# AlexS28/OptiState

Hardware: NVIDIA B200
Metric: kf_trajectory_steps_per_sec (higher is better)
Workload: dtype f64

## Files before the change

### optistate_b200/batch.py

```python
from __future__ import annotations

from dataclasses import dataclass, field
from typing import Dict, Iterable, Optional

import numpy as np
import torch

from . import _native as nv
from .settings import INITIAL_PARAMS

_OUT_ALIASES = {"p_trace": "p_trace_steps", "k_gain": "k_gain_steps", "p_checkpoints": "P_ckpt", "nis": "nis_steps"}
_OUT_SHAPES = {
    "x_steps": lambda T, N, K: (T, 12, N), "x_model_steps": lambda T, N, K: (T, 12, N),
    "p_world_steps": lambda T, N, K: (T, 12, N), "z_steps": lambda T, N, K: (T, 10, N),
    "p_trace_steps": lambda T, N, K: (T, N), "k_gain_steps": lambda T, N, K: (T, N), "nis_steps": lambda T, N, K: (T, N),
    "P_ckpt": lambda T, N, K: (K, 144, N), "x_final": lambda T, N, K: (12, N), "P_final": lambda T, N, K: (144, N),
    "K_final": lambda T, N, K: (120, N), "summary": lambda T, N, K: (nv.SUMMARY_ROWS, N),
}
_ALGOS = {"auto": nv.ALGO_AUTO, "joint": nv.ALGO_JOINT, "sequential": nv.ALGO_SEQUENTIAL}
_ALGO_NAMES = {nv.ALGO_JOINT: "joint", nv.ALGO_SEQUENTIAL: "sequential"}

_GROUP = torch.tensor([0, 0, 0, 1, 2, 3, 0, 0, 0, 1, 2, 3])
_CROSS_GROUP = _GROUP[:, None] != _GROUP[None, :]

SUMMARY_FIELDS = {
    "x_final": slice(0, 12), "p_diag": slice(12, 24), "rmse_truth": slice(24, 36), "rms_dev_nominal": slice(36, 48),
    "mean_nis": 48, "p_trace": 49, "k_gain": 50, "max_nis_sqrt": 51,
}


@dataclass
class KfBatchResult:
    algo: str
    n_traj: int
    n_steps: int
    tensors: Dict[str, torch.Tensor] = field(default_factory=dict)
    status: Optional[torch.Tensor] = None

    def __getattr__(self, name):
        t = self.__dict__.get("tensors", {})
        if name in t:
            return t[name]
        raise AttributeError(name)

    def P_matrix(self, which: str = "P_final") -> torch.Tensor:
        t = self.tensors[which]
        return t.movedim(-1, -2).reshape(*t.shape[:-2], t.shape[-1], 12, 12)

    def summary_field(self, name: str) -> torch.Tensor:
        return self.tensors["summary"][SUMMARY_FIELDS[name]]


def _as_device(a, dtype, device, non_blocking=True):
    if a is None:
        return None
    if isinstance(a, torch.Tensor):
        t = a
    else:
        t = torch.from_numpy(np.ascontiguousarray(a))
    if t.device != device or t.dtype != dtype:
        t = t.to(device=device, dtype=dtype, non_blocking=non_blocking)
    return t.contiguous()


def _stream_tensor(a, C, name, dtype, device):
    t = _as_device(a, dtype, device)
    if t is None:
        return None, None, None
    if t.dim() == 2:
        t = t.unsqueeze(-1)
    if t.dim() != 3 or t.shape[1] != C:
        raise ValueError(f"{name} must have shape [T, {C}, S], got {tuple(t.shape)}")
    return t.contiguous(), t.shape[0], t.shape[2]


def _checked_stream_index(stream_index, N: int, S: int, device) -> torch.Tensor:
    t = _as_device(stream_index, torch.int32, device).reshape(N)
    if N > 0:
        lo, hi = (int(v) for v in torch.aminmax(t))
        if lo < 0 or hi >= S:
            raise ValueError(f"stream_index entries must lie in [0, {S}), got [{lo}, {hi}]")
    return t


def _is_diagonal(m: torch.Tensor) -> bool:
    return bool(torch.count_nonzero(m - torch.diag(torch.diagonal(m))) == 0)


def _noise(a, n, N, name, dtype, device, kind=None):
    t = _as_device(a, dtype, device)
    shp = tuple(t.shape)
    if kind is None:
        if shp == (n,):
            kind = nv.MAT_DIAG
        elif shp == (n, n):
            kind = nv.MAT_DENSE
        elif shp == (n, N):
            kind = nv.MAT_DIAG_PER
        elif shp in ((n * n, N), (n, n, N)):
            kind = nv.MAT_DENSE_PER
        else:
            raise ValueError(f"{name}: unsupported shape {shp} for n={n}, N={N}")
    if kind == nv.MAT_DENSE and _is_diagonal(t.reshape(n, n)):
        t, kind = torch.diagonal(t.reshape(n, n)).contiguous(), nv.MAT_DIAG
    return t.contiguous(), kind


def kf_batch(
    imu, p, dp, contact, f, x0=None, P0=None, Q=None, R=None, *,
    n_traj: Optional[int] = None, dtype: torch.dtype = torch.float64, stream_index=None, stream_offset: int = 0,
    outputs: Iterable[str] = ("x_steps",), ckpt_every: int = 0, truth=None, nominal=None, body_ref=None, z=None,
    algo: str = "auto", cov_model: str = "predict", q_kind=None, r_kind=None, p0_kind=None,
    dt: float = INITIAL_PARAMS.DT_mpc, mass: float = INITIAL_PARAMS.ROBOT_MASS, inertia=None,
    gravity: float = INITIAL_PARAMS.GRAVITY, device=None, out: Optional[Dict[str, torch.Tensor]] = None,
    summary_peers=None, p0_is_symmetric: Optional[bool] = None, structure: str = "auto", packed: bool = True,
) -> KfBatchResult:
    nv.require_cuda()
    ext = nv.ext()
    device = torch.device("cuda", torch.cuda.current_device()) if device is None else torch.device(device)
    if dtype not in (torch.float64, torch.float32):
        raise ValueError("dtype must be torch.float64 or torch.float32")

    tensors: Dict[str, torch.Tensor] = {}
    T = S = None
    for name, arr, C in (("imu", imu, 6), ("p", p, 12), ("dp", dp, 12), ("contact", contact, 4), ("f", f, 12),
                         ("z_in", z, 10), ("body_ref", body_ref, 12), ("truth", truth, 12), ("nominal", nominal, 12)):
        t, tT, tS = _stream_tensor(arr, C, name, dtype, device)
        if t is None:
            continue
        if T is None:
            T, S = tT, tS
        elif (tT, tS) != (T, S):
            raise ValueError(f"{name} has [T,S]=({tT},{tS}), expected ({T},{S})")
        tensors[name] = t
    if T is None:
        raise ValueError("no input streams given")
    N = int(S if n_traj is None else n_traj)
    phases = nv.PHASE_ALL if z is None else (nv.PHASE_PREDICT | nv.PHASE_UPDATE)

    x0_t = _as_device(INITIAL_PARAMS.STARTING_STATE.reshape(12) if x0 is None else x0, dtype, device)
    x0_t = x0_t.reshape(12) if x0_t.numel() == 12 else x0_t.reshape(12, N)
    tensors["x0"] = x0_t.contiguous()
    tensors["Q"], qk = _noise(INITIAL_PARAMS.Q if Q is None else Q, 12, N, "Q", dtype, device, q_kind)
    tensors["R"], rk = _noise(INITIAL_PARAMS.R if R is None else R, 10, N, "R", dtype, device, r_kind)
    pk = nv.MAT_NONE
    p0_symmetric = True
    if structure not in ("auto", "full"):
        raise ValueError("structure must be 'auto' or 'full'")
    flags = nv.FLAG_FULL_COVARIANCE if structure == "full" else 0
    if not packed:
        flags |= nv.FLAG_SCALAR_FP32
    if P0 is not None:
        tensors["P0"], pk = _noise(P0, 12, N, "P0", dtype, device, p0_kind)
        if pk in (nv.MAT_DENSE, nv.MAT_DENSE_PER):
            m = tensors["P0"].reshape(12, 12, -1)
            p0_symmetric = bool(torch.equal(m, m.transpose(0, 1))) if p0_is_symmetric is None else bool(p0_is_symmetric)
            if structure == "auto" and p0_is_symmetric is None and p0_symmetric and cov_model != "mpc":
                if not bool(torch.count_nonzero(m[_CROSS_GROUP.to(device)])):
                    flags |= nv.FLAG_P0_DECOUPLED
    if stream_index is not None:
        tensors["stream_index"] = _checked_stream_index(stream_index, N, S, device)

    want = []
    for o in outputs:
        o = _OUT_ALIASES.get(o, o)
        want.extend(["x_final", "P_final"] if o == "final" else [o])
    n_ckpt = T // ckpt_every if ckpt_every else 0
    for o in want:
        if o not in _OUT_SHAPES:
            raise ValueError(f"unknown output '{o}'")
        shape = _OUT_SHAPES[o](T, N, n_ckpt)
        if o == "summary" and summary_peers is not None:
            if summary_peers.dtype != dtype or summary_peers.n_local != N or summary_peers.device != device:
                raise ValueError("summary_peers was set up for another dtype, device or shard size")
            tensors[o] = summary_peers.tensor
        elif out is not None and o in out:
            if tuple(out[o].shape) != shape or out[o].dtype != dtype:
                raise ValueError(f"out['{o}'] must be {shape} {dtype}")
            tensors[o] = out[o]
        else:
            tensors[o] = torch.empty(shape, dtype=dtype, device=device)
    status = out["status"] if out is not None and "status" in out else torch.zeros(N, dtype=torch.int32, device=device)
    tensors["status"] = status

    cfg = dict(dtype=nv.F64 if dtype == torch.float64 else nv.F32, algo=_ALGOS[algo],
               cov_model=nv.COV_MPC if cov_model == "mpc" else nv.COV_PREDICT, phases=phases, n_traj=N, n_steps=T,
               n_streams=S, stream_offset=int(stream_offset), x0_per_traj=int(x0_t.dim() == 2), p0_kind=pk, q_kind=qk,
               r_kind=rk, ckpt_every=int(ckpt_every), want_K=int("K_final" in want), flags=flags)
    if summary_peers is not None and "summary" in want:
        cfg.update(summary_peers.cfg())
    if cfg["algo"] == nv.ALGO_AUTO:
        probe = dict(cfg, algo=nv.ALGO_SEQUENTIAL)
        cfg["algo"] = nv.ALGO_SEQUENTIAL if (p0_symmetric and ext.kf_resolve_algo(probe) == nv.ALGO_SEQUENTIAL) else nv.ALGO_JOINT
    elif cfg["algo"] == nv.ALGO_SEQUENTIAL and not p0_symmetric:
        raise ValueError("algo='sequential' needs a symmetric P0")
    inertia = np.diag(INITIAL_PARAMS.INERTIA_ROT) if inertia is None else np.asarray(inertia, float).reshape(3)
    consts = dict(dt=float(dt), mass=float(mass), inertia0=float(inertia[0]), inertia1=float(inertia[1]),
                  inertia2=float(inertia[2]), gravity=float(gravity))
    with torch.cuda.device(device):
        ws_bytes = ext.kf_batch(dict(cfg, query_workspace=1), consts, tensors)
        if ws_bytes < 0:
            nv.check(int(ws_bytes), "optistate_kf_workspace_bytes")
        if ws_bytes > 0:
            ws = out.get("workspace") if out is not None else None
            if ws is None or ws.numel() < ws_bytes:
                ws = torch.empty(int(ws_bytes), dtype=torch.uint8, device=device)
            tensors["workspace"] = ws
        nv.check(int(ext.kf_batch(cfg, consts, tensors)), "optistate_kf_batch")
    res = {k: tensors[k] for k in want}
    if summary_peers is not None and "summary" in res:
        res["summary"] = summary_peers.local
    return KfBatchResult(algo=_ALGO_NAMES[cfg["algo"]], n_traj=N, n_steps=T, tensors=res, status=status)


def kf_measure(imu, p, dp, contact, *, dtype: torch.dtype = torch.float64, device=None, want_odom: bool = False):
    nv.require_cuda()
    ext = nv.ext()
    device = torch.device("cuda", torch.cuda.current_device()) if device is None else torch.device(device)
    tensors = {}
    T = S = None
    for name, arr, C in (("imu", imu, 6), ("p", p, 12), ("dp", dp, 12), ("contact", contact, 4)):
        t, tT, tS = _stream_tensor(arr, C, name, dtype, device)
        if T is None:
            T, S = tT, tS
        elif (tT, tS) != (T, S):
            raise ValueError(f"{name} has [T,S]=({tT},{tS}), expected ({T},{S})")
        tensors[name] = t
    tensors["z"] = torch.empty((T, 10, S), dtype=dtype, device=device)
    if want_odom:
        tensors["odom"] = torch.empty((T, 4, S), dtype=dtype, device=device)
    tensors["status"] = torch.zeros(S, dtype=torch.int32, device=device)
    with torch.cuda.device(device):
        nv.check(ext.kf_measure(nv.F64 if dtype == torch.float64 else nv.F32, T, S, tensors), "optistate_kf_measure")
    if want_odom:
        return tensors["z"], tensors["odom"], tensors["status"]
    return tensors["z"], tensors["status"]


def fma_peak(dtype: torch.dtype = torch.float64, fma_per_thread: int = 1 << 16):
    nv.require_cuda()
    return nv.ext().fma_peak(nv.F64 if dtype == torch.float64 else nv.F32, int(fma_per_thread))
```

### optistate_b200/csrc/kf_abi.cu

```cuda
#include <atomic>
#include <cstdlib>
#include <cstring>

#include "kf_features.cuh"
#include "kf_identify.cuh"
#include "kf_launch.cuh"
#include "kf_mpc_params.cuh"

namespace {

std::atomic<long long> g_launches{0};

bool is_diag_kind(int k) { return k == OPTI_KF_MAT_DIAG || k == OPTI_KF_MAT_DIAG_PER; }
bool valid_kind(int k, bool allow_none) { return (k >= (allow_none ? 0 : 1)) && k <= OPTI_KF_MAT_DENSE_PER; }

int validate(const OptiKfDesc *d) {
    if (!d) return OPTI_KF_E_NULL;
    if (d->struct_size != sizeof(OptiKfDesc) || d->abi_version != OPTISTATE_KF_ABI_VERSION) return OPTI_KF_E_VERSION;
    if (d->dtype != OPTI_KF_F64 && d->dtype != OPTI_KF_F32) return OPTI_KF_E_DTYPE;
    if (d->n_traj < 0 || d->n_steps < 0 || d->n_streams <= 0 || d->ckpt_every < 0) return OPTI_KF_E_SHAPE;
    if (d->phases <= 0 || d->phases > OPTI_KF_PHASE_ALL) return OPTI_KF_E_SHAPE;
    if (d->algo < OPTI_KF_ALGO_AUTO || d->algo > OPTI_KF_ALGO_SEQUENTIAL) return OPTI_KF_E_SHAPE;
    if (d->cov_model != OPTI_KF_COV_PREDICT && d->cov_model != OPTI_KF_COV_MPC) return OPTI_KF_E_SHAPE;
    if (!valid_kind(d->q_kind, false) || !valid_kind(d->r_kind, false) || !valid_kind(d->p0_kind, true)) return OPTI_KF_E_SHAPE;
    if (!(d->dt > 0) || !(d->mass > 0) || !(d->inertia[0] > 0) || !(d->inertia[1] > 0) || !(d->inertia[2] > 0)) return OPTI_KF_E_SHAPE;
    const bool work = d->n_traj > 0, steps = work && d->n_steps > 0;
    if (work && (!d->x0 || !d->Q || !d->R)) return OPTI_KF_E_NULL;
    if (work && d->p0_kind != OPTI_KF_MAT_NONE && !d->P0) return OPTI_KF_E_NULL;
    if (steps && (d->phases & OPTI_KF_PHASE_MEASURE) && (!d->imu || !d->p || !d->dp || !d->contact)) return OPTI_KF_E_NULL;
    if (steps && (d->phases & OPTI_KF_PHASE_PREDICT) && (!d->p || !d->f)) return OPTI_KF_E_NULL;
    if (steps && (d->phases & OPTI_KF_PHASE_UPDATE) && !(d->phases & OPTI_KF_PHASE_MEASURE) && !d->z_in) return OPTI_KF_E_NULL;
    if (steps && d->cov_model == OPTI_KF_COV_MPC && (d->phases & OPTI_KF_PHASE_PREDICT) && !d->body_ref) return OPTI_KF_E_NULL;
    if (d->P_ckpt && d->ckpt_every == 0) return OPTI_KF_E_SHAPE;
    if (d->stream_index == nullptr && d->stream_offset < 0) return OPTI_KF_E_SHAPE;
    if (d->summary_ld < 0 || (d->summary_ld > 0 && d->summary_ld < d->n_traj)) return OPTI_KF_E_SHAPE;
    if (d->n_summary_peers < 0 || d->n_summary_peers > OPTI_KF_MAX_PEERS) return OPTI_KF_E_SHAPE;
    if (d->flags & ~(OPTI_KF_FLAG_P0_DECOUPLED | OPTI_KF_FLAG_FULL_COVARIANCE | OPTI_KF_FLAG_SCALAR_FP32 | OPTI_KF_FLAG_STATUS_ACCUMULATE)) return OPTI_KF_E_SHAPE;
    for (int k = 0; k < d->n_summary_peers; ++k)
        if (d->summary && !d->summary_peers[k]) return OPTI_KF_E_NULL;
    return OPTI_KF_OK;
}

bool sequential_ok(const OptiKfDesc *d) {
    return is_diag_kind(d->q_kind) && is_diag_kind(d->r_kind) && d->K_final == nullptr &&
           (d->phases == OPTI_KF_PHASE_ALL || (d->phases == (OPTI_KF_PHASE_PREDICT | OPTI_KF_PHASE_UPDATE) && d->z_in));
}

int resolve(const OptiKfDesc *d) {
    if (d->algo == OPTI_KF_ALGO_JOINT) return OPTI_KF_ALGO_JOINT;
    if (d->algo == OPTI_KF_ALGO_SEQUENTIAL) return sequential_ok(d) ? (int)OPTI_KF_ALGO_SEQUENTIAL : (int)OPTI_KF_E_UNSUPPORTED;
    const bool p0_sym = d->p0_kind == OPTI_KF_MAT_NONE || is_diag_kind(d->p0_kind);
    return (sequential_ok(d) && p0_sym) ? OPTI_KF_ALGO_SEQUENTIAL : OPTI_KF_ALGO_JOINT;
}

template <typename Real>
okf::Params<Real> make_params(const OptiKfDesc *d) {
    okf::Params<Real> p;
    std::memset(&p, 0, sizeof p);
    p.N = d->n_traj; p.T = d->n_steps; p.S = d->n_streams; p.stream_offset = d->stream_offset;
    p.phases = d->phases; p.cov_model = d->cov_model;
    const bool p0_groups = d->p0_kind == OPTI_KF_MAT_NONE || is_diag_kind(d->p0_kind) || (d->flags & OPTI_KF_FLAG_P0_DECOUPLED);
    p.block = (d->cov_model == OPTI_KF_COV_PREDICT && p0_groups && !(d->flags & OPTI_KF_FLAG_FULL_COVARIANCE)) ? 1 : 0;
    p.dt = (Real)d->dt;
    p.dt_over_m = (Real)((1.0 / d->mass) * d->dt);
    p.dt_g = (Real)(d->dt * d->gravity);
    for (int k = 0; k < 3; ++k) p.inv_inertia[k] = (Real)(1.0 / d->inertia[k]);
    p.imu = (const Real *)d->imu; p.p = (const Real *)d->p; p.dp = (const Real *)d->dp;
    p.contact = (const Real *)d->contact; p.f = (const Real *)d->f;
    p.z_in = (d->phases & OPTI_KF_PHASE_MEASURE) ? nullptr : (const Real *)d->z_in;
    p.body_ref = (const Real *)d->body_ref; p.truth = (const Real *)d->truth; p.nominal = (const Real *)d->nominal;
    p.stream_index = d->stream_index;
    p.x0 = (const Real *)d->x0; p.x0_ld = d->x0_per_traj ? d->n_traj : 1; p.x0_inc = d->x0_per_traj ? 1 : 0;
    p.P0 = (const Real *)d->P0; p.p0_kind = d->p0_kind;
    p.Q = (const Real *)d->Q; p.q_kind = d->q_kind;
    p.R = (const Real *)d->R; p.r_kind = d->r_kind;
    p.x_steps = (Real *)d->x_steps; p.x_model_steps = (Real *)d->x_model_steps; p.p_world_steps = (Real *)d->p_world_steps;
    p.z_steps = (Real *)d->z_steps; p.p_trace_steps = (Real *)d->p_trace_steps; p.k_gain_steps = (Real *)d->k_gain_steps;
    p.nis_steps = (Real *)d->nis_steps; p.ckpt_every = d->ckpt_every; p.P_ckpt = (Real *)d->P_ckpt;
    p.x_final = (Real *)d->x_final; p.P_final = (Real *)d->P_final; p.K_final = (Real *)d->K_final;
    p.summary = (Real *)d->summary; p.status = d->status;
    p.summary_ld = d->summary_ld > 0 ? d->summary_ld : d->n_traj;
    p.n_summary_peers = d->summary ? d->n_summary_peers : 0;
    for (int k = 0; k < p.n_summary_peers; ++k) p.summary_peers[k] = (Real *)d->summary_peers[k];
    return p;
}

template <typename Real>
void launch_measure(long long T, long long S, const Real *imu, const Real *p, const Real *dp, const Real *contact, Real *z,
                    Real *odom, uint32_t *status, cudaStream_t stream);

inline bool aligned16(const void *p) { return (reinterpret_cast<uintptr_t>(p) & 15u) == 0; }

size_t seq_workspace_bytes(const OptiKfDesc *d) {
    if (d->phases != OPTI_KF_PHASE_ALL) return 0;
    const size_t esz = d->dtype == OPTI_KF_F64 ? 8 : 4;
    const size_t z_bytes = ((size_t)d->n_steps * okf::NZ * (size_t)d->n_streams * esz + 255) & ~(size_t)255;
    return z_bytes + (((size_t)d->n_streams * sizeof(uint32_t) + 255) & ~(size_t)255);
}

bool tma_layout_ok(const OptiKfDesc *d) {
    if (d->stream_index != nullptr || d->n_steps == 0) return false;
    if (d->n_streams % 32 != 0 || d->stream_offset % 32 != 0) return false;
    if (d->n_steps * 12 >= (1LL << 31)) return false;
    if (!aligned16(d->p) || !aligned16(d->f)) return false;
    if (d->summary && ((d->truth && !aligned16(d->truth)) || (d->nominal && !aligned16(d->nominal)))) return false;
    if (d->cov_model == OPTI_KF_COV_MPC && !aligned16(d->body_ref)) return false;
    return true;
}

inline bool aligned8(const void *p) { return (reinterpret_cast<uintptr_t>(p) & 7u) == 0; }

bool packed_pair_ok(const OptiKfDesc *d) {
    if (d->dtype != OPTI_KF_F32) return false;
    if (d->flags & OPTI_KF_FLAG_SCALAR_FP32) return false;
    if (d->n_traj % 2 != 0 || d->n_streams % 64 != 0 || d->stream_offset % 64 != 0) return false;
    const void *ptrs[] = {d->x0, d->P0, d->Q, d->R, d->x_steps, d->x_model_steps, d->p_world_steps, d->z_steps, d->p_trace_steps,
                          d->k_gain_steps, d->nis_steps, d->P_ckpt, d->x_final, d->P_final, d->summary};
    for (const void *q : ptrs)
        if (q && !aligned8(q)) return false;
    if (d->summary && d->summary_ld % 2 != 0) return false;
    for (int k = 0; k < d->n_summary_peers; ++k)
        if (d->summary && !aligned8(d->summary_peers[k])) return false;
    return true;
}

template <typename Real>
int launch_streamed_t(const OptiKfDesc *d, const okf::Params<typename okf::Lanes<Real>::scalar> &p, cudaStream_t stream) {
    if constexpr (okf::Lanes<Real>::n == 1) {
        if (p.block && p.N <= p.S && p.cov_model == OPTI_KF_COV_PREDICT)
            return d->summary ? okf::launch_seq_tma_lone<Real, true>(p, stream) : okf::launch_seq_tma_lone<Real, false>(p, stream);
    }
    if (p.block) return d->summary ? okf::launch_seq_tma<Real, true, true>(p, stream) : okf::launch_seq_tma<Real, false, true>(p, stream);
    return d->summary ? okf::launch_seq_tma<Real, true, false>(p, stream) : okf::launch_seq_tma<Real, false, false>(p, stream);
}
template <typename Scalar>
int launch_streamed(const OptiKfDesc *d, const okf::Params<Scalar> &p, cudaStream_t stream);
template <>
int launch_streamed<double>(const OptiKfDesc *d, const okf::Params<double> &p, cudaStream_t stream) {
    return launch_streamed_t<double>(d, p, stream);
}
template <>
int launch_streamed<float>(const OptiKfDesc *d, const okf::Params<float> &p, cudaStream_t stream) {
    return packed_pair_ok(d) ? launch_streamed_t<okf::F2>(d, p, stream) : launch_streamed_t<float>(d, p, stream);
}

template <typename Real>
int launch(const OptiKfDesc *d, int algo, cudaStream_t stream) {
    if (d->n_traj == 0) return OPTI_KF_OK;
    okf::Params<Real> p = make_params<Real>(d);
    cudaGetLastError();
    if ((d->flags & OPTI_KF_FLAG_STATUS_ACCUMULATE) && d->status) {
        if (d->stream_index != nullptr || d->n_streams != d->n_traj || d->stream_offset != 0 || d->phases == OPTI_KF_PHASE_ALL) return OPTI_KF_E_UNSUPPORTED;
        p.stream_status = d->status;
    }
    if (algo == OPTI_KF_ALGO_SEQUENTIAL) {
        bool streamed = tma_layout_ok(d);
        if (streamed && d->phases == OPTI_KF_PHASE_ALL) {
            const size_t need = seq_workspace_bytes(d);
            if (d->workspace && d->workspace_bytes >= need && aligned16(d->workspace)) {
                const size_t esz = sizeof(Real);
                const size_t z_bytes = ((size_t)d->n_steps * okf::NZ * (size_t)d->n_streams * esz + 255) & ~(size_t)255;
                Real *z = (Real *)d->workspace;
                uint32_t *sst = (uint32_t *)((unsigned char *)d->workspace + z_bytes);
                if (cudaMemsetAsync(sst, 0, (size_t)d->n_streams * sizeof(uint32_t), stream) != cudaSuccess) return OPTI_KF_E_CUDA;
                launch_measure<Real>(d->n_steps, d->n_streams, p.imu, p.p, p.dp, p.contact, z, nullptr, sst, stream);
                p.z_in = z;
                p.stream_status = sst;
            } else {
                streamed = false;
            }
        } else if (streamed && !aligned16(p.z_in)) {
            streamed = false;
        }
        if (streamed) {
            const int rc = launch_streamed<Real>(d, p, stream);
            if (rc < 0) return rc;
            if (rc == OPTI_KF_OK) {
                g_launches.fetch_add(1, std::memory_order_relaxed);
                return cudaGetLastError() == cudaSuccess ? OPTI_KF_OK : OPTI_KF_E_CUDA;
            }
        }
        const int rc = okf::launch_seq_direct<Real>(p, stream);
        if (rc < 0) return rc;
    } else {
        const int rc = okf::launch_joint<Real>(p, stream);
        if (rc < 0) return rc;
    }
    g_launches.fetch_add(1, std::memory_order_relaxed);
    return cudaGetLastError() == cudaSuccess ? OPTI_KF_OK : OPTI_KF_E_CUDA;
}

template <typename Real>
__global__ void __launch_bounds__(256) kf_measure_kernel(long long T, long long S, const Real *__restrict__ imu,
                                                         const Real *__restrict__ p, const Real *__restrict__ dp,
                                                         const Real *__restrict__ contact, Real *__restrict__ z,
                                                         Real *__restrict__ odom, uint32_t *__restrict__ status) {
    const long long idx = (long long)blockIdx.x * blockDim.x + threadIdx.x;
    if (idx >= T * S) return;
    const long long t = idx / S, s = idx % S;
    Real im[6], pp[12], dd[12], cc[4], zz[okf::NZ];
#pragma unroll
    for (int c = 0; c < 6; ++c) im[c] = imu[(t * 6 + c) * S + s];
#pragma unroll
    for (int c = 0; c < 12; ++c) { pp[c] = p[(t * 12 + c) * S + s]; dd[c] = dp[(t * 12 + c) * S + s]; }
#pragma unroll
    for (int c = 0; c < 4; ++c) cc[c] = contact[(t * 4 + c) * S + s];
    const bool all_swing = okf::form_measurement(im, pp, dd, cc, zz);
    if (z) {
#pragma unroll
        for (int c = 0; c < okf::NZ; ++c) z[(t * okf::NZ + c) * S + s] = zz[c];
    }
    if (odom) {
        odom[(t * 4 + 0) * S + s] = zz[3];
        odom[(t * 4 + 1) * S + s] = zz[7];
        odom[(t * 4 + 2) * S + s] = zz[8];
        odom[(t * 4 + 3) * S + s] = zz[9];
    }
    if (status && all_swing) atomicOr(status + s, (uint32_t)OPTI_KF_ST_ALL_SWING);
}

template <typename Real>
void launch_measure(long long T, long long S, const Real *imu, const Real *p, const Real *dp, const Real *contact, Real *z,
                    Real *odom, uint32_t *status, cudaStream_t stream) {
    const long long total = T * S;
    if (total == 0) return;
    kf_measure_kernel<Real><<<(unsigned)((total + 255) / 256), 256, 0, stream>>>(T, S, imu, p, dp, contact, z, odom, status);
    g_launches.fetch_add(1, std::memory_order_relaxed);
}

template <typename Real>
__global__ void __launch_bounds__(256) fma_peak_kernel(long long iters, Real seed, Real *sink) {
    Real a[16];
    const Real m = Real(0.999) + seed * Real(1e-9), c = Real(1e-3) * (Real)(threadIdx.x & 7);
#pragma unroll
    for (int k = 0; k < 16; ++k) a[k] = seed + (Real)k;
    for (long long it = 0; it < iters; ++it) {
#pragma unroll
        for (int k = 0; k < 16; ++k) a[k] = a[k] * m + c;
    }
    Real s = Real(0);
#pragma unroll
    for (int k = 0; k < 16; ++k) s += a[k];
    if (s == Real(-12345.678)) sink[blockIdx.x * blockDim.x + threadIdx.x] = s;
}

template <typename Real>
int fma_peak(long long fma_per_thread, double *flops_out, double *seconds_out, cudaStream_t stream) {
    int dev = 0, sms = 0;
    if (cudaGetDevice(&dev) != cudaSuccess) return OPTI_KF_E_NO_DEVICE;
    cudaDeviceGetAttribute(&sms, cudaDevAttrMultiProcessorCount, dev);
    const int blocks = sms * 8, threads = 256;
    const long long iters = (fma_per_thread + 15) / 16;
    cudaEvent_t e0, e1;
    if (cudaEventCreate(&e0) != cudaSuccess || cudaEventCreate(&e1) != cudaSuccess) return OPTI_KF_E_CUDA;
    fma_peak_kernel<Real><<<blocks, threads, 0, stream>>>(iters / 8 + 1, Real(1), nullptr);
    cudaEventRecord(e0, stream);
    fma_peak_kernel<Real><<<blocks, threads, 0, stream>>>(iters, Real(1), nullptr);
    cudaEventRecord(e1, stream);
    g_launches.fetch_add(2, std::memory_order_relaxed);
    if (cudaEventSynchronize(e1) != cudaSuccess) { cudaEventDestroy(e0); cudaEventDestroy(e1); return OPTI_KF_E_CUDA; }
    float ms = 0.f;
    cudaEventElapsedTime(&ms, e0, e1);
    cudaEventDestroy(e0); cudaEventDestroy(e1);
    const double fma = (double)iters * 16.0 * (double)blocks * (double)threads;
    if (flops_out) *flops_out = 2.0 * fma / ((double)ms * 1e-3);
    if (seconds_out) *seconds_out = (double)ms * 1e-3;
    return OPTI_KF_OK;
}

template <typename Real>
int identify_noise(const OptiKfIdentifyDesc *d, cudaStream_t stream) {
    okf::Params<Real> p;
    std::memset(&p, 0, sizeof p);
    p.N = d->n_traj; p.T = d->n_steps; p.S = d->n_streams; p.stream_offset = d->stream_offset; p.stream_index = d->stream_index;
    p.dt = (Real)d->dt;
    p.dt_over_m = (Real)((1.0 / d->mass) * d->dt);
    p.dt_g = (Real)(d->dt * d->gravity);
    for (int k = 0; k < 3; ++k) p.inv_inertia[k] = (Real)(1.0 / d->inertia[k]);
    p.imu = (const Real *)d->imu; p.p = (const Real *)d->p; p.dp = (const Real *)d->dp;
    p.contact = (const Real *)d->contact; p.f = (const Real *)d->f; p.status = d->status;
    const long long pairs = (d->n_steps - 1) * d->n_traj;
    okf::kf_identify_residuals_kernel<Real><<<(unsigned)((pairs + 127) / 128), 128, 0, stream>>>(p, (const Real *)d->gt, d->alias_last_measurement,
                                                                                                  (Real *)d->scratch);
    const long long comps = (long long)okf::IDENT_ROWS * d->n_traj;
    okf::kf_identify_variance_kernel<Real><<<(unsigned)((comps + 127) / 128), 128, 0, stream>>>(d->n_traj, d->n_steps - 1, (const Real *)d->scratch,
                                                                                                 (Real *)d->q_diag, (Real *)d->r_diag);
    g_launches.fetch_add(2, std::memory_order_relaxed);
    return cudaGetLastError() == cudaSuccess ? OPTI_KF_OK : OPTI_KF_E_CUDA;
}

}

extern "C" {

int optistate_kf_abi_version(void) { return OPTISTATE_KF_ABI_VERSION; }
size_t optistate_kf_desc_size(void) { return sizeof(OptiKfDesc); }
int64_t optistate_kf_launch_count(void) { return (int64_t)g_launches.load(std::memory_order_relaxed); }

int optistate_kf_resolve_algo(const OptiKfDesc *desc) {
    const int rc = validate(desc);
    return rc != OPTI_KF_OK ? rc : resolve(desc);
}

int optistate_kf_workspace_bytes(const OptiKfDesc *desc, size_t *bytes_out) {
    const int rc = validate(desc);
    if (rc != OPTI_KF_OK) return rc;
    if (!bytes_out) return OPTI_KF_E_NULL;
    const int algo = resolve(desc);
    if (algo < 0) return algo;
    *bytes_out = (algo == OPTI_KF_ALGO_SEQUENTIAL && tma_layout_ok(desc)) ? seq_workspace_bytes(desc) : 0;
    return OPTI_KF_OK;
}

int optistate_kf_batch(const OptiKfDesc *desc, void *cuda_stream) {
    const int rc = validate(desc);
    if (rc != OPTI_KF_OK) return rc;
    const int algo = resolve(desc);
    if (algo < 0) return algo;
    cudaStream_t stream = (cudaStream_t)cuda_stream;
    return desc->dtype == OPTI_KF_F64 ? launch<double>(desc, algo, stream) : launch<float>(desc, algo, stream);
}

int optistate_kf_batch_f64(const OptiKfDesc *desc, void *cuda_stream) {
    if (desc && desc->dtype != OPTI_KF_F64) return OPTI_KF_E_DTYPE;
    return optistate_kf_batch(desc, cuda_stream);
}

int optistate_kf_batch_f32(const OptiKfDesc *desc, void *cuda_stream) {
    if (desc && desc->dtype != OPTI_KF_F32) return OPTI_KF_E_DTYPE;
    return optistate_kf_batch(desc, cuda_stream);
}

int optistate_kf_measure(const OptiKfMeasureDesc *d, void *cuda_stream) {
    if (!d) return OPTI_KF_E_NULL;
    if (d->struct_size != sizeof(OptiKfMeasureDesc) || d->abi_version != OPTISTATE_KF_ABI_VERSION) return OPTI_KF_E_VERSION;
    if (d->dtype != OPTI_KF_F64 && d->dtype != OPTI_KF_F32) return OPTI_KF_E_DTYPE;
    if (d->n_steps < 0 || d->n_streams <= 0) return OPTI_KF_E_SHAPE;
    if (!d->imu || !d->p || !d->dp || !d->contact || (!d->z && !d->odom)) return OPTI_KF_E_NULL;
    const long long total = d->n_steps * d->n_streams;
    if (total == 0) return OPTI_KF_OK;
    cudaStream_t stream = (cudaStream_t)cuda_stream;
    cudaGetLastError();
    if (d->dtype == OPTI_KF_F64)
        launch_measure<double>(d->n_steps, d->n_streams, (const double *)d->imu, (const double *)d->p, (const double *)d->dp,
                               (const double *)d->contact, (double *)d->z, (double *)d->odom, d->status, stream);
    else
        launch_measure<float>(d->n_steps, d->n_streams, (const float *)d->imu, (const float *)d->p, (const float *)d->dp,
                              (const float *)d->contact, (float *)d->z, (float *)d->odom, d->status, stream);
    return cudaGetLastError() == cudaSuccess ? OPTI_KF_OK : OPTI_KF_E_CUDA;
}

int optistate_fma_peak(int dtype, int64_t fma_per_thread, double *flops_per_s_out, double *seconds_out, void *cuda_stream) {
    if (fma_per_thread <= 0) return OPTI_KF_E_SHAPE;
    cudaStream_t stream = (cudaStream_t)cuda_stream;
    if (dtype == OPTI_KF_F64) return fma_peak<double>(fma_per_thread, flops_per_s_out, seconds_out, stream);
    if (dtype == OPTI_KF_F32) return fma_peak<float>(fma_per_thread, flops_per_s_out, seconds_out, stream);
    return OPTI_KF_E_DTYPE;
}

int optistate_kf_features(const OptiKfFeatureDesc *d, void *cuda_stream) {
    if (!d) return OPTI_KF_E_NULL;
    if (d->struct_size != sizeof(OptiKfFeatureDesc) || d->abi_version != OPTISTATE_KF_ABI_VERSION) return OPTI_KF_E_VERSION;
    if (d->dtype != OPTI_KF_F64 && d->dtype != OPTI_KF_F32) return OPTI_KF_E_DTYPE;
    if (d->n_traj < 0 || d->n_steps < 0 || d->n_streams <= 0) return OPTI_KF_E_SHAPE;
    if ((d->n_steps + okf::FEAT_STEPS - 1) / okf::FEAT_STEPS > 65535) return OPTI_KF_E_SHAPE;
    if (d->stream_index == nullptr && d->stream_offset < 0) return OPTI_KF_E_SHAPE;
    if (!d->x_steps || !d->p_world_steps || !d->imu || !d->f || !d->dp || !d->rows) return OPTI_KF_E_NULL;
    if (d->n_traj == 0 || d->n_steps == 0) return OPTI_KF_OK;
    cudaStream_t stream = (cudaStream_t)cuda_stream;
    const dim3 grid((unsigned)((d->n_traj + okf::FEAT_TRAJ - 1) / okf::FEAT_TRAJ), (unsigned)((d->n_steps + okf::FEAT_STEPS - 1) / okf::FEAT_STEPS));
    cudaGetLastError();
    if (d->dtype == OPTI_KF_F64)
        okf::kf_features_kernel<double><<<grid, 256, 0, stream>>>(d->n_traj, d->n_steps, d->n_streams, d->stream_offset, d->stream_index,
                                                                  (const double *)d->x_steps, (const double *)d->p_world_steps,
                                                                  (const double *)d->imu, (const double *)d->imu_acc, (const double *)d->f,
                                                                  (const double *)d->dp, (double *)d->rows);
    else
        okf::kf_features_kernel<float><<<grid, 256, 0, stream>>>(d->n_traj, d->n_steps, d->n_streams, d->stream_offset, d->stream_index,
                                                                 (const float *)d->x_steps, (const float *)d->p_world_steps,
                                                                 (const float *)d->imu, (const float *)d->imu_acc, (const float *)d->f,
                                                                 (const float *)d->dp, (float *)d->rows);
    g_launches.fetch_add(1, std::memory_order_relaxed);
    return cudaGetLastError() == cudaSuccess ? OPTI_KF_OK : OPTI_KF_E_CUDA;
}

static const int kMinmaxBlocks = 592;
static int sm_count() {
    int dev = 0, n = 0;
    if (cudaGetDevice(&dev) != cudaSuccess || cudaDeviceGetAttribute(&n, cudaDevAttrMultiProcessorCount, dev) != cudaSuccess || n <= 0) n = 148;
    return n;
}

size_t optistate_kf_minmax_scratch_bytes(int dtype, int32_t n_cols) {
    return (size_t)kMinmaxBlocks * 2 * (size_t)(n_cols > 0 ? n_cols : 0) * (dtype == OPTI_KF_F64 ? 8 : 4);
}

int optistate_kf_minmax(int dtype, const void *rows, int64_t n_rows, int32_t n_cols, void *min_out, void *max_out, void *scratch,
                        size_t scratch_bytes, void *cuda_stream) {
    if (dtype != OPTI_KF_F64 && dtype != OPTI_KF_F32) return OPTI_KF_E_DTYPE;
    if (!rows || !min_out || !max_out || !scratch) return OPTI_KF_E_NULL;
    if (n_rows <= 0 || n_cols <= 0 || n_cols > 256 || scratch_bytes < optistate_kf_minmax_scratch_bytes(dtype, n_cols)) return OPTI_KF_E_SHAPE;
    cudaStream_t stream = (cudaStream_t)cuda_stream;
    cudaGetLastError();
    const int nblk = 4 * sm_count() < kMinmaxBlocks ? 4 * sm_count() : kMinmaxBlocks;
    if (dtype == OPTI_KF_F64) {
        okf::kf_minmax_partial_kernel<double><<<nblk, 256, 2 * 256 * sizeof(double), stream>>>((const double *)rows, n_rows, n_cols, (double *)scratch);
        okf::kf_minmax_final_kernel<double><<<1, 256, 0, stream>>>((const double *)scratch, nblk, n_cols, (double *)min_out, (double *)max_out);
    } else {
        okf::kf_minmax_partial_kernel<float><<<nblk, 256, 2 * 256 * sizeof(float), stream>>>((const float *)rows, n_rows, n_cols, (float *)scratch);
        okf::kf_minmax_final_kernel<float><<<1, 256, 0, stream>>>((const float *)scratch, nblk, n_cols, (float *)min_out, (float *)max_out);
    }
    g_launches.fetch_add(2, std::memory_order_relaxed);
    return cudaGetLastError() == cudaSuccess ? OPTI_KF_OK : OPTI_KF_E_CUDA;
}

size_t optistate_kf_windows_scratch_bytes(int64_t n_groups, int64_t rows_per_group, int32_t n_cols, int32_t n_latent) {
    if (n_groups <= 0 || rows_per_group <= 0 || n_cols <= 0 || n_latent < 0) return 0;
    return (size_t)n_groups * (size_t)rows_per_group * (size_t)(n_cols + n_latent) * sizeof(float);
}

int optistate_kf_windows(int dtype, const void *rows, const float *latent, const void *mn, const void *mx, int64_t n_groups,
                         int64_t rows_per_group, int32_t n_cols, int32_t n_latent, int32_t seq_len, float *out, void *scratch,
                         size_t scratch_bytes, void *cuda_stream) {
    if (dtype != OPTI_KF_F64 && dtype != OPTI_KF_F32) return OPTI_KF_E_DTYPE;
    if (!rows || !mn || !mx || !out || !scratch || (n_latent > 0 && !latent)) return OPTI_KF_E_NULL;
    if (n_groups <= 0 || seq_len <= 0 || rows_per_group < seq_len || n_cols <= 0 || n_latent < 0) return OPTI_KF_E_SHAPE;
    if (scratch_bytes < optistate_kf_windows_scratch_bytes(n_groups, rows_per_group, n_cols, n_latent)) return OPTI_KF_E_SHAPE;
    cudaStream_t stream = (cudaStream_t)cuda_stream;
    const long long n_rows = n_groups * rows_per_group;
    const int width = n_cols + n_latent;
    float *full = (float *)scratch;
    cudaGetLastError();
    const unsigned nb = (unsigned)sm_count() * 16;
    if (dtype == OPTI_KF_F64)
        okf::kf_normalise_rows_kernel<double><<<nb, 256, 0, stream>>>((const double *)rows, latent, (const double *)mn, (const double *)mx,
                                                                      n_rows, n_cols, n_latent, full);
    else
        okf::kf_normalise_rows_kernel<float><<<nb, 256, 0, stream>>>((const float *)rows, latent, (const float *)mn, (const float *)mx, n_rows,
                                                                     n_cols, n_latent, full);
    const bool vec4 = (width % 4 == 0) && ((reinterpret_cast<uintptr_t>(full) | reinterpret_cast<uintptr_t>(out)) & 15u) == 0;
    if (vec4)
        okf::kf_windows_copy_kernel<float4><<<nb, dim3(64, 4), 0, stream>>>((const float4 *)full, rows_per_group, n_groups, width / 4, seq_len, (float4 *)out);
    else
        okf::kf_windows_copy_kernel<float><<<nb, dim3(64, 4), 0, stream>>>(full, rows_per_group, n_groups, width, seq_len, out);
    g_launches.fetch_add(2, std::memory_order_relaxed);
    return cudaGetLastError() == cudaSuccess ? OPTI_KF_OK : OPTI_KF_E_CUDA;
}

size_t optistate_kf_identify_scratch_bytes(int dtype, int64_t n_traj, int64_t n_steps) {
    if (n_traj <= 0 || n_steps < 2) return 0;
    return (size_t)(n_steps - 1) * okf::IDENT_ROWS * (size_t)n_traj * (dtype == OPTI_KF_F64 ? 8 : 4);
}

int optistate_kf_identify_noise(const OptiKfIdentifyDesc *d, void *cuda_stream) {
    if (!d) return OPTI_KF_E_NULL;
    if (d->struct_size != sizeof(OptiKfIdentifyDesc) || d->abi_version != OPTISTATE_KF_ABI_VERSION) return OPTI_KF_E_VERSION;
    if (d->dtype != OPTI_KF_F64 && d->dtype != OPTI_KF_F32) return OPTI_KF_E_DTYPE;
    if (d->n_traj <= 0 || d->n_steps < 2 || d->n_streams <= 0) return OPTI_KF_E_SHAPE;
    if (d->stream_index == nullptr && d->stream_offset < 0) return OPTI_KF_E_SHAPE;
    if (!(d->dt > 0) || !(d->mass > 0) || !(d->inertia[0] > 0) || !(d->inertia[1] > 0) || !(d->inertia[2] > 0)) return OPTI_KF_E_SHAPE;
    if (!d->gt || !d->imu || !d->p || !d->dp || !d->contact || !d->f || !d->q_diag || !d->r_diag || !d->scratch) return OPTI_KF_E_NULL;
    if (d->scratch_bytes < optistate_kf_identify_scratch_bytes(d->dtype, d->n_traj, d->n_steps)) return OPTI_KF_E_SHAPE;
    cudaGetLastError();
    cudaStream_t stream = (cudaStream_t)cuda_stream;
    return d->dtype == OPTI_KF_F64 ? identify_noise<double>(d, stream) : identify_noise<float>(d, stream);
}

int optistate_kf_mpc_forces(const OptiKfMpcDesc *d, void *cuda_stream) {
    if (!d) return OPTI_KF_E_NULL;
    if (d->struct_size != sizeof(OptiKfMpcDesc) || d->abi_version != OPTISTATE_KF_ABI_VERSION) return OPTI_KF_E_VERSION;
    if (d->dtype != OPTI_KF_F64) return OPTI_KF_E_DTYPE;
    if (d->n_problems < 0 || d->max_free_legs < 0 || d->max_free_legs > 4) return OPTI_KF_E_SHAPE;
    if (!(d->dt > 0) || !(d->mass > 0) || !(d->inertia[0] > 0) || !(d->inertia[1] > 0) || !(d->inertia[2] > 0) || !(d->mu > 0) ||
        !(d->fz_max > 0) || !(d->w_force > 0))
        return OPTI_KF_E_SHAPE;
    for (int k = 0; k < 12; ++k)
        if (!(d->w_state[k] >= 0)) return OPTI_KF_E_SHAPE;
    if (d->n_problems == 0) return OPTI_KF_OK;
    if (!d->x || !d->body_ref || !d->p || !d->contact || !d->forces || !d->status) return OPTI_KF_E_NULL;
    if ((d->warm_set == nullptr) != (d->warm_mult == nullptr)) return OPTI_KF_E_NULL;
    okf::MpcParams p;
    std::memset(&p, 0, sizeof p);
    p.N = d->n_problems;
    p.max_legs = d->max_free_legs == 0 ? 4 : d->max_free_legs;
    p.x = (const double *)d->x; p.body_ref = (const double *)d->body_ref; p.p = (const double *)d->p;
    p.contact = (const double *)d->contact; p.forces = (double *)d->forces; p.status = d->status;
    p.warm_set = d->warm_set; p.warm_mult = (double *)d->warm_mult;
    if (d->solver != 0 && d->solver != 1) return OPTI_KF_E_SHAPE;
    p.solver = d->solver;
    p.max_changes = d->max_changes > 0 ? d->max_changes : 0;
    p.dt = d->dt; p.inv_mass = 1.0 / d->mass; p.gravity = d->gravity; p.mu = d->mu; p.fz_max = d->fz_max; p.w_force = d->w_force;
    for (int k = 0; k < 3; ++k) p.inv_inertia[k] = 1.0 / d->inertia[k];
    for (int k = 0; k < 12; ++k) p.w_state[k] = d->w_state[k];
    cudaGetLastError();
    const int rc = okf::launch_mpc(p, (cudaStream_t)cuda_stream);
    if (rc < 0) return rc;
    g_launches.fetch_add(1, std::memory_order_relaxed);
    return cudaGetLastError() == cudaSuccess ? OPTI_KF_OK : OPTI_KF_E_CUDA;
}

int optistate_kf_peer_alloc(size_t bytes, void **dev_ptr_out) {
    if (!dev_ptr_out || bytes == 0) return OPTI_KF_E_NULL;
    *dev_ptr_out = nullptr;
    return cudaMalloc(dev_ptr_out, bytes) == cudaSuccess ? (int)OPTI_KF_OK : (cudaGetLastError(), (int)OPTI_KF_E_CUDA);
}

int optistate_kf_peer_free(void *dev_ptr) {
    if (!dev_ptr) return OPTI_KF_OK;
    return cudaFree(dev_ptr) == cudaSuccess ? (int)OPTI_KF_OK : (cudaGetLastError(), (int)OPTI_KF_E_CUDA);
}

int optistate_kf_peer_export(void *dev_ptr, unsigned char handle_out[OPTI_KF_PEER_HANDLE_BYTES]) {
    static_assert(sizeof(cudaIpcMemHandle_t) <= OPTI_KF_PEER_HANDLE_BYTES, "handle does not fit");
    if (!dev_ptr || !handle_out) return OPTI_KF_E_NULL;
    cudaIpcMemHandle_t h;
    if (cudaIpcGetMemHandle(&h, dev_ptr) != cudaSuccess) { cudaGetLastError(); return OPTI_KF_E_CUDA; }
    std::memset(handle_out, 0, OPTI_KF_PEER_HANDLE_BYTES);
    std::memcpy(handle_out, &h, sizeof h);
    return OPTI_KF_OK;
}

int optistate_kf_peer_open(const unsigned char handle[OPTI_KF_PEER_HANDLE_BYTES], void **peer_ptr_out) {
    if (!handle || !peer_ptr_out) return OPTI_KF_E_NULL;
    cudaIpcMemHandle_t h;
    std::memcpy(&h, handle, sizeof h);
    *peer_ptr_out = nullptr;
    if (cudaIpcOpenMemHandle(peer_ptr_out, h, cudaIpcMemLazyEnablePeerAccess) != cudaSuccess) { cudaGetLastError(); return OPTI_KF_E_CUDA; }
    return OPTI_KF_OK;
}

int optistate_kf_peer_close(void *peer_ptr) {
    if (!peer_ptr) return OPTI_KF_OK;
    return cudaIpcCloseMemHandle(peer_ptr) == cudaSuccess ? (int)OPTI_KF_OK : (cudaGetLastError(), (int)OPTI_KF_E_CUDA);
}

const char *optistate_kf_strerror(int code) {
    switch (code) {
        case OPTI_KF_OK: return "ok";
        case OPTI_KF_E_NULL: return "descriptor or a required pointer is NULL";
        case OPTI_KF_E_VERSION: return "descriptor size / ABI version mismatch";
        case OPTI_KF_E_DTYPE: return "unsupported or mismatching dtype";
        case OPTI_KF_E_SHAPE: return "invalid sizes, kinds or constants";
        case OPTI_KF_E_UNSUPPORTED: return "combination not supported by the requested algo";
        case OPTI_KF_E_CUDA: return "CUDA runtime error at launch";
        case OPTI_KF_E_NO_DEVICE: return "no CUDA device";
        default: return "unknown error";
    }
}

}
```

### optistate_b200/csrc/kf_closed_loop.cu

```cuda
#include <cuda_runtime.h>

#include <cstring>

#include "../../include/optistate_kf.h"

namespace {

constexpr size_t kAlign = 256;
inline size_t up(size_t b) { return (b + kAlign - 1) & ~(kAlign - 1); }

struct Layout {
    size_t z, p0, p1, fh, wset, wmult, mst, total;
    Layout(int64_t N, int64_t T) {
        size_t o = 0;
        z = o; o += up((size_t)T * 10 * N * 8);
        p0 = o; o += up((size_t)144 * N * 8);
        p1 = o; o += up((size_t)144 * N * 8);
        fh = o; o += up((size_t)OPTI_KF_MPC_HORIZON * 12 * N * 8);
        wset = o; o += up((size_t)OPTI_KF_MPC_HORIZON * N * 4);
        wmult = o; o += up((size_t)OPTI_KF_MPC_HORIZON * 4 * 5 * N * 8);
        mst = o; o += up((size_t)N * 4);
        total = o;
    }
};

__global__ void broadcast_state_kernel(const double *x, double *out, long long N) {
    const long long i = (long long)blockIdx.x * blockDim.x + threadIdx.x;
    if (i < 12 * N) out[i] = x[i / N];
}

}

extern "C" {

size_t optistate_kf_closed_loop_workspace_bytes(int64_t n_traj, int64_t n_steps) {
    if (n_traj <= 0 || n_steps <= 0) return 0;
    return Layout(n_traj, n_steps).total;
}

int optistate_kf_closed_loop(const OptiKfClosedLoopDesc *d, void *cuda_stream) {
    if (!d) return OPTI_KF_E_NULL;
    if (d->struct_size != sizeof(OptiKfClosedLoopDesc) || d->abi_version != OPTISTATE_KF_ABI_VERSION) return OPTI_KF_E_VERSION;
    if (d->dtype != OPTI_KF_F64) return OPTI_KF_E_DTYPE;
    if (d->n_traj < 0 || d->n_steps < 0 || d->max_free_legs < 0 || d->max_free_legs > 4) return OPTI_KF_E_SHAPE;
    if (d->n_traj == 0 || d->n_steps == 0) return OPTI_KF_OK;
    if (!d->imu || !d->p || !d->dp || !d->contact || !d->body_ref || !d->x0 || !d->Q || !d->R || !d->x_steps || !d->workspace) return OPTI_KF_E_NULL;
    const bool diag_q = d->q_kind == OPTI_KF_MAT_DIAG || d->q_kind == OPTI_KF_MAT_DIAG_PER;
    const bool diag_r = d->r_kind == OPTI_KF_MAT_DIAG || d->r_kind == OPTI_KF_MAT_DIAG_PER;
    if (!diag_q || !diag_r) return OPTI_KF_E_UNSUPPORTED;
    if (d->p0_kind != OPTI_KF_MAT_NONE && !d->P0) return OPTI_KF_E_NULL;
    const int64_t N = d->n_traj, T = d->n_steps;
    const Layout L(N, T);
    if (d->workspace_bytes < L.total || (reinterpret_cast<uintptr_t>(d->workspace) & 15u)) return OPTI_KF_E_SHAPE;
    cudaStream_t stream = (cudaStream_t)cuda_stream;
    unsigned char *ws = (unsigned char *)d->workspace;
    double *z = (double *)(ws + L.z), *Pbuf[2] = {(double *)(ws + L.p0), (double *)(ws + L.p1)}, *fh = (double *)(ws + L.fh);
    uint32_t *wset = (uint32_t *)(ws + L.wset), *mst_scratch = (uint32_t *)(ws + L.mst);
    double *wmult = (double *)(ws + L.wmult);
    if (cudaMemsetAsync(wset, 0, (size_t)OPTI_KF_MPC_HORIZON * N * 4, stream) != cudaSuccess) return OPTI_KF_E_CUDA;
    if (d->status && cudaMemsetAsync(d->status, 0, (size_t)N * 4, stream) != cudaSuccess) return OPTI_KF_E_CUDA;

    OptiKfMeasureDesc m;
    std::memset(&m, 0, sizeof m);
    m.struct_size = sizeof m; m.abi_version = OPTISTATE_KF_ABI_VERSION; m.dtype = OPTI_KF_F64;
    m.n_steps = T; m.n_streams = N;
    m.imu = d->imu; m.p = d->p; m.dp = d->dp; m.contact = d->contact; m.z = z; m.status = d->status;
    int rc = optistate_kf_measure(&m, stream);
    if (rc != OPTI_KF_OK) return rc;

    OptiKfMpcDesc q;
    std::memset(&q, 0, sizeof q);
    q.struct_size = sizeof q; q.abi_version = OPTISTATE_KF_ABI_VERSION; q.dtype = OPTI_KF_F64;
    q.max_free_legs = d->max_free_legs; q.n_problems = N;
    q.forces = fh;
    q.dt = d->dt; q.mass = d->mass; q.gravity = d->gravity; q.mu = d->mu; q.fz_max = d->fz_max; q.w_force = d->w_force;
    for (int k = 0; k < 3; ++k) q.inertia[k] = d->inertia[k];
    for (int k = 0; k < 12; ++k) q.w_state[k] = d->w_state[k];
    q.solver = d->solver; q.max_changes = d->max_changes;
    if (d->warm_start) { q.warm_set = wset; q.warm_mult = wmult; }

    OptiKfDesc f;
    std::memset(&f, 0, sizeof f);
    f.struct_size = sizeof f; f.abi_version = OPTISTATE_KF_ABI_VERSION; f.dtype = OPTI_KF_F64;
    f.algo = OPTI_KF_ALGO_SEQUENTIAL; f.cov_model = OPTI_KF_COV_MPC; f.phases = OPTI_KF_PHASE_PREDICT | OPTI_KF_PHASE_UPDATE;
    f.n_traj = N; f.n_steps = 1; f.n_streams = N; f.stream_offset = 0;
    f.dt = d->dt; f.mass = d->mass; f.gravity = d->gravity;
    for (int k = 0; k < 3; ++k) f.inertia[k] = d->inertia[k];
    f.q_kind = d->q_kind; f.r_kind = d->r_kind; f.Q = d->Q; f.R = d->R;
    f.status = d->status;
    f.flags = d->status ? OPTI_KF_FLAG_STATUS_ACCUMULATE : 0;

    const double *x_cur = (const double *)d->x0;
    int x_per = d->x0_per_traj;
    for (int64_t t = 0; t < T; ++t) {
        const double *p_t = (const double *)d->p + t * 12 * N;
        const double *x_mpc = x_cur;
        if (!x_per) {
            double *xb = Pbuf[1];
            broadcast_state_kernel<<<(unsigned)((12 * N + 255) / 256), 256, 0, stream>>>(x_cur, xb, N);
            x_mpc = xb;
        }
        q.x = x_mpc;
        q.body_ref = (const double *)d->body_ref + t * OPTI_KF_MPC_HORIZON * 12 * N;
        q.p = p_t;
        q.contact = (const double *)d->contact + t * 4 * N;
        q.status = d->mpc_status ? d->mpc_status + t * N : mst_scratch;
        rc = optistate_kf_mpc_forces(&q, stream);
        if (rc != OPTI_KF_OK) return rc;
        if (d->forces && cudaMemcpyAsync((double *)d->forces + t * 12 * N, fh, (size_t)12 * N * 8, cudaMemcpyDeviceToDevice, stream) != cudaSuccess)
            return OPTI_KF_E_CUDA;
        f.p = p_t;
        f.f = fh;
        f.z_in = z + t * 10 * N;
        f.body_ref = q.body_ref;
        f.x0 = x_cur; f.x0_per_traj = x_per;
        if (t == 0) { f.p0_kind = d->p0_kind; f.P0 = d->P0; }
        else { f.p0_kind = OPTI_KF_MAT_DENSE_PER; f.P0 = Pbuf[(t - 1) & 1]; }
        f.x_final = (double *)d->x_steps + t * 12 * N;
        f.P_final = Pbuf[t & 1];
        f.p_world_steps = d->p_world_steps ? (double *)d->p_world_steps + t * 12 * N : nullptr;
        rc = optistate_kf_batch(&f, stream);
        if (rc != OPTI_KF_OK) return rc;
        x_cur = (const double *)f.x_final;
        x_per = 1;
    }
    return OPTI_KF_OK;
}

}
```

### optistate_b200/csrc/kf_common.cuh

```cuda
#pragma once

#include <cuda_runtime.h>
#include <stdint.h>

#include "../../include/optistate_kf.h"
#include "kf_arith.cuh"

namespace okf {

constexpr int NX = OPTI_KF_NX;
constexpr int NZ = OPTI_KF_NZ;
__host__ __device__ constexpr int sel(int j) { return j < 3 ? j : j + 2; }

template <typename Real>
struct Params {
    long long N, T, S, stream_offset;
    int phases, cov_model;
    int block;
    Real dt, dt_over_m, dt_g, inv_inertia[3];
    const Real *imu, *p, *dp, *contact, *f, *z_in, *body_ref, *truth, *nominal;
    const int32_t *stream_index;
    const Real *x0; long long x0_ld; int x0_inc;
    const Real *P0; int p0_kind;
    const Real *Q; int q_kind;
    const Real *R; int r_kind;
    Real *x_steps, *x_model_steps, *p_world_steps, *z_steps, *p_trace_steps, *k_gain_steps, *nis_steps;
    long long ckpt_every;
    Real *P_ckpt, *x_final, *P_final, *K_final, *summary;
    uint32_t *status;
    const uint32_t *stream_status;
    long long summary_ld;
    int n_summary_peers;
    Real *summary_peers[OPTI_KF_MAX_PEERS];
};

template <typename Real, typename V>
__device__ __forceinline__ void st_summary(const Params<Real> &prm, int row, long long i, V v) {
    const long long idx = (long long)row * prm.summary_ld + i;
    st_traj(prm.summary, idx, v);
    for (int k = 0; k < prm.n_summary_peers; ++k) st_traj(prm.summary_peers[k], idx, v);
}

template <typename Real> __device__ __forceinline__ void sincos_full(Real a, Real &s, Real &c);
template <> __device__ __forceinline__ void sincos_full<double>(double x, double &s, double &c) {
    const double q = rint(x * 6.36619772367581382433e-01);
    double r = fma(-q, 1.57079632673412561417e+00, x);
    r = fma(-q, 6.07710050630396597660e-11, r);
    r = fma(-q, 2.02226624871116645580e-21, r);
    r = fma(-q, 8.47842766036889956997e-32, r);
    const double z = r * r;
    double ps = fma(z, 1.58969099521155010221e-10, -2.50507602534068634195e-08);
    ps = fma(z, ps, 2.75573137070700676789e-06);
    ps = fma(z, ps, -1.98412698298579493134e-04);
    ps = fma(z, ps, 8.33333333332248946124e-03);
    ps = fma(z, ps, -1.66666666666666324348e-01);
    const double sr = fma(z * r, ps, r);
    double pc = fma(z, -1.13596475577881948265e-11, 2.08757232129817482790e-09);
    pc = fma(z, pc, -2.75573143513906633035e-07);
    pc = fma(z, pc, 2.48015872894767294178e-05);
    pc = fma(z, pc, -1.38888888888741095749e-03);
    pc = fma(z, pc, 4.16666666666666019037e-02);
    const double cr = 1.0 - fma(0.5, z, -(z * (z * pc)));
    const int n = __double2int_rn(q);
    const double s0 = (n & 1) ? cr : sr, c0 = (n & 1) ? sr : cr;
    s = (n & 2) ? -s0 : s0;
    c = ((n + 1) & 2) ? -c0 : c0;
}
template <> __device__ __forceinline__ void sincos_full<float>(float x, float &s, float &c) {
    const float q = rintf(x * 0.636619772367581343f);
    float r = fmaf(-q, 1.5703125f, x);
    r = fmaf(-q, 4.837512969970703125e-4f, r);
    r = fmaf(-q, 7.54978995489188216e-8f, r);
    const float z = r * r;
    float ps = fmaf(z, -1.9515295891e-4f, 8.3321608736e-3f);
    ps = fmaf(z, ps, -1.6666654611e-1f);
    const float sr = fmaf(z * r, ps, r);
    float pc = fmaf(z, 2.443315711809948e-5f, -1.388731625493765e-3f);
    pc = fmaf(z, pc, 4.166664568298827e-2f);
    const float cr = 1.0f - fmaf(0.5f, z, -(z * (z * pc)));
    const int n = __float2int_rn(q);
    const float s0 = (n & 1) ? cr : sr, c0 = (n & 1) ? sr : cr;
    s = (n & 2) ? -s0 : s0;
    c = ((n + 1) & 2) ? -c0 : c0;
}
template <> __device__ __forceinline__ void sincos_full<F2>(F2 a, F2 &s, F2 &c) {
    sincos_full<float>(a.v.x, s.v.x, c.v.x);
    sincos_full<float>(a.v.y, s.v.y, c.v.y);
}

__device__ __forceinline__ double mul_rn(double a, double b) { return __dmul_rn(a, b); }
__device__ __forceinline__ float mul_rn(float a, float b) { return __fmul_rn(a, b); }
__device__ __forceinline__ double add_rn(double a, double b) { return __dadd_rn(a, b); }
__device__ __forceinline__ float add_rn(float a, float b) { return __fadd_rn(a, b); }
__device__ __forceinline__ F2 mul_rn(F2 a, F2 b) { return a * b; }
__device__ __forceinline__ F2 add_rn(F2 a, F2 b) { return a + b; }

template <typename Real>
__device__ __forceinline__ void rot_zyx(Real a, Real b, Real c, Real (&R)[9]) {
    Real sa, ca, sb, cb, sc, cc;
    sincos_full(a, sa, ca);
    sincos_full(b, sb, cb);
    sincos_full(c, sc, cc);
    const Real sbsa = mul_rn(sb, sa), sbca = mul_rn(sb, ca);
    R[0] = mul_rn(cc, cb);
    R[1] = add_rn(mul_rn(cc, sbsa), -mul_rn(sc, ca));
    R[2] = add_rn(mul_rn(cc, sbca), mul_rn(sc, sa));
    R[3] = mul_rn(sc, cb);
    R[4] = add_rn(mul_rn(sc, sbsa), mul_rn(cc, ca));
    R[5] = add_rn(mul_rn(sc, sbca), -mul_rn(cc, sa));
    R[6] = -sb;
    R[7] = mul_rn(cb, sa);
    R[8] = mul_rn(cb, ca);
}

__device__ __forceinline__ void trunc_rt(const double (&R)[9], const double *, double (&Tm)[9], bool &any) {
    any = false;
#pragma unroll
    for (int i = 0; i < 3; ++i)
#pragma unroll
        for (int j = 0; j < 3; ++j) {
            const double v = trunc(R[3 * j + i]);
            Tm[3 * i + j] = v;
            any |= (v != 0.0);
        }
}
__device__ __forceinline__ void trunc_rt(const float (&R)[9], const float *ang, float (&Tm)[9], bool &any) {
    float m = 0.f;
#pragma unroll
    for (int k = 0; k < 9; ++k) { m = fmaxf(m, fabsf(R[k])); Tm[k] = 0.f; }
    any = false;
    if (m >= 1.0f - 9.5367431640625e-7f) {
        double Rd[9], Td[9];
        rot_zyx<double>((double)ang[0], (double)ang[1], (double)ang[2], Rd);
        trunc_rt(Rd, nullptr, Td, any);
#pragma unroll
        for (int k = 0; k < 9; ++k) Tm[k] = (float)Td[k];
    }
}

template <typename Real>
__device__ __forceinline__ bool form_measurement(const Real (&imu)[6], const Real (&p)[12], const Real (&dp)[12],
                                                 const Real (&contact)[4], Real (&z)[NZ]) {
    Real nc = 0, sx = 0, sy = 0, sv = 0, sz = 0;
#pragma unroll
    for (int l = 0; l < 4; ++l) {
        nc += contact[l];
        const bool stance = (contact[l] == Real(1)), swing = (contact[l] == Real(0));
        sx += stance ? dp[3 * l] : Real(0);
        sy += stance ? dp[3 * l + 1] : Real(0);
        sz += stance ? p[3 * l + 2] : Real(0);
        sv += swing ? dp[3 * l + 2] : Real(0);
    }
    const bool all_swing = (nc == Real(0));
    Real vb[3] = {Real(0), Real(0), Real(0)}, zo = Real(0);
    if (!all_swing) {
        vb[0] = -sx / nc; vb[1] = -sy / nc; vb[2] = -sv / nc; zo = -sz / nc;
    }
    Real Ri[9];
    rot_zyx(imu[0], imu[1], imu[2], Ri);
    z[0] = imu[0]; z[1] = imu[1]; z[2] = imu[2]; z[3] = zo;
    z[4] = imu[3]; z[5] = imu[4]; z[6] = imu[5];
#pragma unroll
    for (int i = 0; i < 3; ++i) z[7 + i] = Ri[3 * i] * vb[0] + Ri[3 * i + 1] * vb[1] + Ri[3 * i + 2] * vb[2];
    return all_swing;
}

template <typename Real>
__device__ __forceinline__ void propagate_mean(const Params<Real> &P, Real (&x)[NX], Real (&p)[12], const Real (&f)[12],
                                               Real (&R)[9]) {
    rot_zyx(x[0], x[1], x[2], R);
    Real Tm[9];
    bool any;
    trunc_rt(R, x, Tm, any);
    Real tau[3] = {Real(0), Real(0), Real(0)}, fs[3] = {Real(0), Real(0), Real(0)};
#pragma unroll
    for (int l = 0; l < 4; ++l) {
        const Real a = p[3 * l], b = p[3 * l + 1], c = p[3 * l + 2];
        const Real pw0 = R[0] * a + R[1] * b + R[2] * c;
        const Real pw1 = R[3] * a + R[4] * b + R[5] * c;
        const Real pw2 = R[6] * a + R[7] * b + R[8] * c;
        p[3 * l] = pw0; p[3 * l + 1] = pw1; p[3 * l + 2] = pw2;
        const Real f0 = f[3 * l], f1 = f[3 * l + 1], f2 = f[3 * l + 2];
        tau[0] += pw1 * f2 - pw2 * f1;
        tau[1] += pw2 * f0 - pw0 * f2;
        tau[2] += pw0 * f1 - pw1 * f0;
        fs[0] += f0; fs[1] += f1; fs[2] += f2;
    }
    Real u[3];
#pragma unroll
    for (int k = 0; k < 3; ++k) u[k] = (R[k] * tau[0] + R[3 + k] * tau[1] + R[6 + k] * tau[2]) * P.inv_inertia[k];
    Real xn[NX];
#pragma unroll
    for (int i = 0; i < 3; ++i) {
        Real dth = Real(0);
        if (any) dth = P.dt * (Tm[3 * i] * x[6] + Tm[3 * i + 1] * x[7] + Tm[3 * i + 2] * x[8]);
        xn[i] = x[i] + dth;
        xn[3 + i] = x[3 + i] + P.dt * x[9 + i];
        xn[6 + i] = x[6 + i] + P.dt * (R[3 * i] * u[0] + R[3 * i + 1] * u[1] + R[3 * i + 2] * u[2]);
        xn[9 + i] = x[9 + i] + P.dt_over_m * fs[i];
    }
    xn[11] += P.dt_g;
#pragma unroll
    for (int i = 0; i < NX; ++i) x[i] = xn[i];
}

template <typename Real>
__device__ __forceinline__ long long stream_of(const Params<Real> &P, long long i) {
    return P.stream_index ? (long long)P.stream_index[i] : (i + P.stream_offset) % P.S;
}

template <typename Real> __device__ __forceinline__ Real ld_stream(const Real *p) { return __ldg(p); }
template <typename Real> __device__ __forceinline__ void st_stream(Real *p, Real v) { __stcs(p, v); }

template <typename Real> __device__ __forceinline__ bool finite_all(const Real (&x)[NX]) {
    bool ok = true;
#pragma unroll
    for (int i = 0; i < NX; ++i) ok &= (fabs((double)x[i]) <= 1.79e308) && (x[i] == x[i]);
    return ok;
}

}
```

### optistate_b200/csrc/kf_seq.cuh

```cuda
#pragma once

#include "kf_seq_core.cuh"

namespace okf {

constexpr int SEQ_NOISE_ROWS = 22;

template <typename Real, bool kSummary, bool kMpc, bool kBlock = false>
__global__ void __launch_bounds__(128) kf_seq_kernel(const __grid_constant__ Params<Real> prm) {
    extern __shared__ __align__(128) unsigned char smem_raw[];
    Real *noise = reinterpret_cast<Real *>(smem_raw);
    const int nt = blockDim.x;
    const long long i = (long long)blockIdx.x * nt + threadIdx.x;
    if (i >= prm.N) return;
    const long long N = prm.N, S = prm.S;
    const long long s = stream_of(prm, i);
    Real *q = noise + threadIdx.x, *r = noise + 12 * nt + threadIdx.x;
#pragma unroll
    for (int c = 0; c < NX; ++c) q[c * nt] = prm.q_kind == OPTI_KF_MAT_DIAG ? prm.Q[c] : prm.Q[c * N + i];
#pragma unroll
    for (int c = 0; c < NZ; ++c) r[c * nt] = prm.r_kind == OPTI_KF_MAT_DIAG ? prm.R[c] : prm.R[c * N + i];

    Real x[NX], P[NP];
#pragma unroll
    for (int c = 0; c < NX; ++c) x[c] = prm.x0[c * prm.x0_ld + i * prm.x0_inc];
#pragma unroll
    for (int a = 0; a < NX; ++a)
#pragma unroll
        for (int b = 0; b <= a; ++b) {
            Real v = Real(0);
            if (cpl<kBlock>(a, b)) switch (prm.p0_kind) {
                case OPTI_KF_MAT_NONE: v = (a == b) ? q[a * nt] : Real(0); break;
                case OPTI_KF_MAT_DIAG: v = (a == b) ? prm.P0[a] : Real(0); break;
                case OPTI_KF_MAT_DIAG_PER: v = (a == b) ? prm.P0[a * N + i] : Real(0); break;
                case OPTI_KF_MAT_DENSE: v = prm.P0[a * NX + b]; break;
                default: v = prm.P0[(long long)(a * NX + b) * N + i]; break;
            }
            P[tri(a, b)] = v;
        }

    uint32_t status[1] = {0};
    Real ptrace = Real(0), kgain = Real(0), ymax = Real(0);
    double acc_truth[kSummary ? NX : 1], acc_nom[kSummary ? NX : 1], acc_nis = 0.0;
    if (kSummary) {
#pragma unroll
        for (int c = 0; c < NX; ++c) { acc_truth[c] = 0.0; acc_nom[c] = 0.0; }
    }

    Real Rm[9];
    rot_zyx(x[0], x[1], x[2], Rm);
    bool any_trunc = may_truncate(Rm);

    for (long long t = 0; t < prm.T; ++t) {
        const bool last = t + 1 == prm.T;
        Real z[NZ], pf[12], ff[12];
#pragma unroll
        for (int c = 0; c < 12; ++c) {
            pf[c] = ld_stream(prm.p + (t * 12 + c) * S + s);
            ff[c] = ld_stream(prm.f + (t * 12 + c) * S + s);
        }
        if (prm.z_in) {
#pragma unroll
            for (int c = 0; c < NZ; ++c) z[c] = ld_stream(prm.z_in + (t * NZ + c) * S + s);
        } else {
            Real imu[6], dp[12], contact[4];
#pragma unroll
            for (int c = 0; c < 6; ++c) imu[c] = ld_stream(prm.imu + (t * 6 + c) * S + s);
#pragma unroll
            for (int c = 0; c < 12; ++c) dp[c] = ld_stream(prm.dp + (t * 12 + c) * S + s);
#pragma unroll
            for (int c = 0; c < 4; ++c) contact[c] = ld_stream(prm.contact + (t * 4 + c) * S + s);
            if (form_measurement(imu, pf, dp, contact, z)) status[0] |= OPTI_KF_ST_ALL_SWING;
        }

        propagate_mean_with_R<1>(prm, x, pf, ff, Rm, any_trunc, prm.p_world_steps, (t * 12) * N + i, N);
        if (prm.x_model_steps) {
#pragma unroll
            for (int c = 0; c < NX; ++c) st_stream(prm.x_model_steps + (t * NX + c) * N + i, x[c]);
        }
        if (prm.z_steps) {
#pragma unroll
            for (int c = 0; c < NZ; ++c) st_stream(prm.z_steps + (t * NZ + c) * N + i, z[c]);
        }

        if constexpr (kMpc) {
            Real Rb[9], E[9];
            rot_zyx(ld_stream(prm.body_ref + (t * 12 + 0) * S + s), ld_stream(prm.body_ref + (t * 12 + 1) * S + s),
                    ld_stream(prm.body_ref + (t * 12 + 2) * S + s), Rb);
#pragma unroll
            for (int a = 0; a < 3; ++a)
#pragma unroll
                for (int k = 0; k < 3; ++k) E[3 * a + k] = exp_minus_one(prm.dt * Rb[3 * k + a]);
            cov_predict_mpc_sym(P, E, exp_minus_one(prm.dt), q, nt);
        } else {
            cov_predict_sym<kBlock>(P, Rm, prm.dt, q, nt);
        }

        Real nis = Real(0), inv, inv_n;
        {
            const Real s0 = P[tri(0, 0)] + r[0];
            note_bad_pivot(s0, status, OPTI_KF_ST_NOT_PD);
            inv = rcp_(s0);
        }
        auto nothing = [] {};
        fold_pipelined<0, kBlock>(P, x, z[0], r[0 * nt], r[1 * nt], inv, inv_n, nis, status, nothing); inv = inv_n;
        fold_pipelined<1, kBlock>(P, x, z[1], r[1 * nt], r[2 * nt], inv, inv_n, nis, status, nothing); inv = inv_n;
        fold_pipelined<2, kBlock>(P, x, z[2], r[2 * nt], r[3 * nt], inv, inv_n, nis, status, nothing); inv = inv_n;
        fold_pipelined<3, kBlock>(P, x, z[3], r[3 * nt], r[4 * nt], inv, inv_n, nis, status, nothing); inv = inv_n;
        fold_pipelined<4, kBlock>(P, x, z[4], r[4 * nt], r[5 * nt], inv, inv_n, nis, status, nothing); inv = inv_n;
        fold_pipelined<5, kBlock>(P, x, z[5], r[5 * nt], r[6 * nt], inv, inv_n, nis, status, nothing); inv = inv_n;
        fold_pipelined<6, kBlock>(P, x, z[6], r[6 * nt], r[7 * nt], inv, inv_n, nis, status, nothing); inv = inv_n;
        fold_pipelined<7, kBlock>(P, x, z[7], r[7 * nt], r[8 * nt], inv, inv_n, nis, status, nothing); inv = inv_n;
        fold_pipelined<8, kBlock>(P, x, z[8], r[8 * nt], r[9 * nt], inv, inv_n, nis, status, nothing); inv = inv_n;
        fold_pipelined<9, kBlock>(P, x, z[9], r[9 * nt], r[9 * nt], inv, inv_n, nis, status, [&] {
            rot_zyx(x[0], x[1], x[2], Rm);
            any_trunc = may_truncate(Rm);
        });

        ymax = max_(ymax, nis);
        ptrace = Real(0);
#pragma unroll
        for (int c = 0; c < NX; ++c) ptrace += P[tri(c, c)];
        if (prm.k_gain_steps != nullptr || (last && prm.summary != nullptr)) {
            kgain = gain_trace<kBlock>(P, r, nt);
        }
        if (prm.x_steps) {
#pragma unroll
            for (int c = 0; c < NX; ++c) st_stream(prm.x_steps + (t * NX + c) * N + i, x[c]);
        }
        if (prm.p_trace_steps) st_stream(prm.p_trace_steps + t * N + i, ptrace);
        if (prm.k_gain_steps) st_stream(prm.k_gain_steps + t * N + i, kgain);
        if (prm.nis_steps) st_stream(prm.nis_steps + t * N + i, nis);
        if (kSummary) {
            acc_nis += (double)nis;
            if (prm.truth) {
#pragma unroll
                for (int c = 0; c < NX; ++c) acc_truth[c] = err_acc(acc_truth[c], x[c], ld_stream(prm.truth + (t * NX + c) * S + s));
            }
            if (prm.nominal) {
#pragma unroll
                for (int c = 0; c < NX; ++c) acc_nom[c] = err_acc(acc_nom[c], x[c], ld_stream(prm.nominal + (t * NX + c) * S + s));
            }
        }
        if (prm.P_ckpt && prm.ckpt_every > 0 && (t + 1) % prm.ckpt_every == 0) {
            Real *dst = prm.P_ckpt + ((t + 1) / prm.ckpt_every - 1) * (long long)(NX * NX) * N + i;
#pragma unroll
            for (int a = 0; a < NX; ++a)
#pragma unroll
                for (int b = 0; b < NX; ++b) dst[(long long)(a * NX + b) * N] = cpl<kBlock>(a, b) ? P[tri(a, b)] : Real(0);
        }
    }

#pragma unroll
    for (int c = 0; c < NX; ++c) note_nonfinite(x[c], status, OPTI_KF_ST_NONFINITE);
    if (prm.x_final) {
#pragma unroll
        for (int c = 0; c < NX; ++c) prm.x_final[c * N + i] = x[c];
    }
    if (prm.P_final) {
#pragma unroll
        for (int a = 0; a < NX; ++a)
#pragma unroll
            for (int b = 0; b < NX; ++b) prm.P_final[(long long)(a * NX + b) * N + i] = cpl<kBlock>(a, b) ? P[tri(a, b)] : Real(0);
    }
    if (kSummary && prm.summary) {
        const double invT = prm.T > 0 ? 1.0 / (double)prm.T : 0.0;
#pragma unroll
        for (int c = 0; c < NX; ++c) {
            st_summary(prm, c, i, x[c]);
            st_summary(prm, 12 + c, i, P[tri(c, c)]);
            st_summary(prm, 24 + c, i, (Real)sqrt(acc_truth[c] * invT));
            st_summary(prm, 36 + c, i, (Real)sqrt(acc_nom[c] * invT));
        }
        st_summary(prm, 48, i, (Real)(acc_nis * invT));
        st_summary(prm, 49, i, ptrace);
        st_summary(prm, 50, i, kgain);
        st_summary(prm, 51, i, (Real)sqrt((double)ymax));
    }
    if (prm.status) prm.status[i] = status[0] | (prm.stream_status ? prm.stream_status[s] : 0u);
}

}
```

### optistate_b200/csrc/kf_seq_core.cuh

```cuda
#pragma once

#include "kf_common.cuh"

namespace okf {

__host__ __device__ constexpr int tri(int i, int j) { return i >= j ? i * (i + 1) / 2 + j : j * (j + 1) / 2 + i; }
constexpr int NP = 78;

__host__ __device__ constexpr int grp(int i) { return (i < 3 || (i >= 6 && i < 9)) ? 0 : 1 + (i % 3); }
template <bool kBlock>
__host__ __device__ constexpr bool cpl(int i, int j) { return !kBlock || grp(i) == grp(j); }

template <bool kBlock = false, typename Real, typename Scalar>
__device__ __forceinline__ void cov_predict_sym(Real (&P)[NP], const Real (&R)[9], Scalar dt_s, const Real *q, int qs) {
    constexpr int a = 0, b = 3, c = 6, d = 9;
    const Real dt = Real(dt_s);
    Real A[9];
#pragma unroll
    for (int i = 0; i < 3; ++i)
#pragma unroll
        for (int k = 0; k < 3; ++k) A[3 * i + k] = dt * R[3 * k + i];
#pragma unroll
    for (int i = 0; i < 3; ++i)
#pragma unroll
        for (int j = 0; j <= i; ++j) {
            Real s = P[tri(a + i, a + j)];
#pragma unroll
            for (int k = 0; k < 3; ++k) s = fma_(A[3 * i + k], P[tri(c + k, a + j)], s);
            P[tri(a + i, a + j)] = s;
        }
#pragma unroll
    for (int i = 0; i < 3; ++i)
#pragma unroll
        for (int j = 0; j < 3; ++j)
            if (cpl<kBlock>(b + i, a + j)) P[tri(b + i, a + j)] = fma_(dt, P[tri(d + i, a + j)], P[tri(b + i, a + j)]);
#pragma unroll
    for (int i = 0; i < 3; ++i)
#pragma unroll
        for (int j = 0; j <= i; ++j)
            if (cpl<kBlock>(b + i, b + j)) P[tri(b + i, b + j)] = fma_(dt, P[tri(d + i, b + j)], P[tri(b + i, b + j)]);
#pragma unroll
    for (int i = 0; i < 3; ++i)
#pragma unroll
        for (int j = 0; j < 3; ++j) {
            Real s = P[tri(c + i, a + j)];
#pragma unroll
            for (int k = 0; k < 3; ++k) s = fma_(P[tri(c + i, c + k)], A[3 * j + k], s);
            P[tri(c + i, a + j)] = s;
            if (cpl<kBlock>(d + i, a + j)) {
                Real u = P[tri(d + i, a + j)];
#pragma unroll
                for (int k = 0; k < 3; ++k) u = fma_(P[tri(d + i, c + k)], A[3 * j + k], u);
                P[tri(d + i, a + j)] = u;
            }
        }
#pragma unroll
    for (int i = 0; i < 3; ++i)
#pragma unroll
        for (int j = 0; j < 3; ++j) {
            if (cpl<kBlock>(c + i, b + j)) P[tri(c + i, b + j)] = fma_(dt, P[tri(d + j, c + i)], P[tri(c + i, b + j)]);
            if (cpl<kBlock>(d + i, b + j)) P[tri(d + i, b + j)] = fma_(dt, P[tri(d + i, d + j)], P[tri(d + i, b + j)]);
        }
#pragma unroll
    for (int i = 0; i < 3; ++i)
#pragma unroll
        for (int j = 0; j <= i; ++j) {
            Real s = P[tri(a + i, a + j)];
#pragma unroll
            for (int k = 0; k < 3; ++k) s = fma_(P[tri(c + k, a + i)], A[3 * j + k], s);
            P[tri(a + i, a + j)] = s;
        }
#pragma unroll
    for (int i = 0; i < 3; ++i)
#pragma unroll
        for (int j = 0; j < 3; ++j)
            if (cpl<kBlock>(b + i, a + j)) {
                Real s = P[tri(b + i, a + j)];
#pragma unroll
                for (int k = 0; k < 3; ++k) s = fma_(P[tri(c + k, b + i)], A[3 * j + k], s);
                P[tri(b + i, a + j)] = s;
            }
#pragma unroll
    for (int i = 0; i < 3; ++i)
#pragma unroll
        for (int j = 0; j <= i; ++j)
            if (cpl<kBlock>(b + i, b + j)) P[tri(b + i, b + j)] = fma_(dt, P[tri(d + j, b + i)], P[tri(b + i, b + j)]);
#pragma unroll
    for (int i = 0; i < NX; ++i) P[tri(i, i)] += q[i * qs];
}

__device__ __forceinline__ double exp_minus_one(double x) { return exp(x) - 1.0; }
__device__ __forceinline__ float exp_minus_one(float x) { return (float)(exp((double)x) - 1.0); }
__device__ __forceinline__ F2 exp_minus_one(F2 x) { return F2(exp_minus_one(x.v.x), exp_minus_one(x.v.y)); }

template <typename Real>
__device__ __forceinline__ void cov_predict_mpc_sym(Real (&P)[NP], const Real (&E)[9], Real e1, const Real *q, int qs) {
    Real w[NX];
#pragma unroll
    for (int i = 0; i < NX; ++i) {
        Real acc = P[tri(i, 0)];
#pragma unroll
        for (int j = 1; j < NX; ++j) acc += P[tri(i, j)];
        w[i] = acc;
    }
    Real s = w[0];
#pragma unroll
    for (int i = 1; i < NX; ++i) s += w[i];
    Real v[6];
#pragma unroll
    for (int a = 0; a < 3; ++a) {
        v[a] = fma_(E[3 * a + 2], w[8], fma_(E[3 * a + 1], w[7], E[3 * a] * w[6]));
        v[3 + a] = e1 * w[9 + a];
    }
    Real U[9];
#pragma unroll
    for (int a = 0; a < 3; ++a)
#pragma unroll
        for (int kk = 0; kk < 3; ++kk)
            U[3 * a + kk] = fma_(E[3 * a + 2], P[tri(8, 6 + kk)], fma_(E[3 * a + 1], P[tri(7, 6 + kk)], E[3 * a] * P[tri(6, 6 + kk)]));
    Real G[21];
#pragma unroll
    for (int a = 0; a < 3; ++a) {
#pragma unroll
        for (int b = 0; b <= a; ++b) G[tri(a, b)] = fma_(U[3 * a + 2], E[3 * b + 2], fma_(U[3 * a + 1], E[3 * b + 1], U[3 * a] * E[3 * b]));
#pragma unroll
        for (int b = 0; b < 3; ++b)
            G[tri(3 + a, b)] = e1 * fma_(P[tri(9 + a, 8)], E[3 * b + 2], fma_(P[tri(9 + a, 7)], E[3 * b + 1], P[tri(9 + a, 6)] * E[3 * b]));
#pragma unroll
        for (int b = 0; b <= a; ++b) G[tri(3 + a, 3 + b)] = (e1 * e1) * P[tri(9 + a, 9 + b)];
    }
#pragma unroll
    for (int i = 0; i < NX; ++i)
#pragma unroll
        for (int j = 0; j <= i; ++j) {
            Real val = s;
            if (i < 6) val += v[i];
            if (j < 6) val += v[j];
            if (i < 6) val += G[tri(i, j)];
            if (i == j) val += q[i * qs];
            P[tri(i, j)] = val;
        }
}

template <int J, bool kBlock = false, typename Real, int L, typename Mid>
__device__ __forceinline__ void fold_pipelined(Real (&P)[NP], Real (&x)[NX], Real zj, Real rj, Real r_next, Real inv, Real &inv_next,
                                               Real &nis, uint32_t (&status)[L], Mid mid) {
    constexpr int k = sel(J);
    constexpr int kn = (J + 1 < NZ) ? sel(J + 1) : -1;
    if constexpr (kn >= 0) {
        Real pnn = P[tri(kn, kn)];
        if constexpr (cpl<kBlock>(kn, k)) {
            const Real wn = P[tri(kn, k)] * inv;
            pnn = fnma_(wn, P[tri(kn, k)], pnn);
            P[tri(kn, kn)] = pnn;
        }
        const Real s = pnn + r_next;
        note_bad_pivot(s, status, OPTI_KF_ST_NOT_PD);
        inv_next = rcp_(s);
    }
    const Real y = zj - x[k];
    const Real g = inv * y;
    nis = fma_(y, g, nis);
#pragma unroll
    for (int i = 0; i < NX; ++i)
        if (cpl<kBlock>(i, k)) x[i] = fma_(P[tri(i, k)], g, x[i]);
    mid();
#pragma unroll
    for (int i = 0; i < NX; ++i) {
        if (i == k || !cpl<kBlock>(i, k)) continue;
        const Real w = P[tri(i, k)] * inv;
#pragma unroll
        for (int j = 0; j <= i; ++j) {
            if (j == k || !cpl<kBlock>(j, k) || (i == kn && j == kn)) continue;
            P[tri(i, j)] = fnma_(w, P[tri(j, k)], P[tri(i, j)]);
        }
    }
    const Real cfac = rj * inv;
#pragma unroll
    for (int i = 0; i < NX; ++i)
        if (cpl<kBlock>(i, k)) P[tri(i, k)] *= cfac;
}

template <bool kBlock = false, typename Real>
__device__ __forceinline__ Real gain_trace(const Real (&P)[NP], const Real *r, int stride) {
    Real g = Real(0);
#pragma unroll
    for (int j = 0; j < NZ; ++j)
        if (cpl<kBlock>(j, sel(j))) g = fma_(P[tri(j, sel(j))], rcp_(r[j * stride]), g);
    return g;
}

template <bool kBlock = false, typename Real>
__device__ __forceinline__ Real gain_trace_rinv(const Real (&P)[NP], const Real *rinv, int stride) {
    Real g0 = Real(0), g1 = Real(0);
#pragma unroll
    for (int j = 0; j < NZ; j += 2) {
        if (cpl<kBlock>(j, sel(j))) g0 = fma_(P[tri(j, sel(j))], rinv[j * stride], g0);
        if (cpl<kBlock>(j + 1, sel(j + 1))) g1 = fma_(P[tri(j + 1, sel(j + 1))], rinv[(j + 1) * stride], g1);
    }
    return g0 + g1;
}

template <typename Real>
__device__ __forceinline__ bool may_truncate(const Real (&R)[9]) {
    using S = typename Lanes<Real>::scalar;
    int m = 0;
#pragma unroll
    for (int k = 0; k < 9; ++k) m = max(m, abs_bits(R[k]));
    return m >= (sizeof(S) == 8 ? 0x3ff00000 : 0x3f7ffff0);
}

template <int STRIDE, typename Real, typename Scalar>
__device__ __forceinline__ void propagate_mean_with_R(const Params<Scalar> &prm, Real (&x)[NX], const Real *pin, const Real *fin,
                                                      const Real (&R)[9], bool any_trunc, Scalar *pw_out, long long pw_idx, long long pw_stride) {
    constexpr int L = Lanes<Real>::n;
    Real tau[3] = {Real(0), Real(0), Real(0)}, fs[3] = {Real(0), Real(0), Real(0)};
#pragma unroll
    for (int l = 0; l < 4; ++l) {
        const Real a = pin[(3 * l) * STRIDE], b = pin[(3 * l + 1) * STRIDE], c = pin[(3 * l + 2) * STRIDE];
        const Real pw0 = fma_(R[2], c, fma_(R[1], b, R[0] * a));
        const Real pw1 = fma_(R[5], c, fma_(R[4], b, R[3] * a));
        const Real pw2 = fma_(R[8], c, fma_(R[7], b, R[6] * a));
        if (pw_out) {
            st_traj(pw_out, pw_idx + (3 * l) * pw_stride, pw0);
            st_traj(pw_out, pw_idx + (3 * l + 1) * pw_stride, pw1);
            st_traj(pw_out, pw_idx + (3 * l + 2) * pw_stride, pw2);
        }
        const Real f0 = fin[(3 * l) * STRIDE], f1 = fin[(3 * l + 1) * STRIDE], f2 = fin[(3 * l + 2) * STRIDE];
        tau[0] += fnma_(pw2, f1, pw1 * f2);
        tau[1] += fnma_(pw0, f2, pw2 * f0);
        tau[2] += fnma_(pw1, f0, pw0 * f1);
        fs[0] += f0; fs[1] += f1; fs[2] += f2;
    }
    Real u[3];
#pragma unroll
    for (int k = 0; k < 3; ++k) u[k] = fma_(R[6 + k], tau[2], fma_(R[3 + k], tau[1], R[k] * tau[0])) * Real(prm.inv_inertia[k]);
    Real dth[3] = {Real(0), Real(0), Real(0)};
    if (any_trunc) {
#pragma unroll
        for (int ln = 0; ln < L; ++ln) {
            Scalar Rs[9], Ts[9], ang[3];
            bool any;
#pragma unroll
            for (int k = 0; k < 9; ++k) Rs[k] = lane_get(R[k], ln);
#pragma unroll
            for (int k = 0; k < 3; ++k) ang[k] = lane_get(x[k], ln);
            trunc_rt(Rs, ang, Ts, any);
#pragma unroll
            for (int i = 0; i < 3; ++i)
                lane_set(dth[i], ln, prm.dt * (Ts[3 * i] * lane_get(x[6], ln) + Ts[3 * i + 1] * lane_get(x[7], ln) + Ts[3 * i + 2] * lane_get(x[8], ln)));
        }
    }
    const Real dt = Real(prm.dt);
    Real xn[NX];
#pragma unroll
    for (int i = 0; i < 3; ++i) {
        xn[i] = x[i] + dth[i];
        xn[3 + i] = fma_(dt, x[9 + i], x[3 + i]);
        xn[6 + i] = fma_(dt, fma_(R[3 * i + 2], u[2], fma_(R[3 * i + 1], u[1], R[3 * i] * u[0])), x[6 + i]);
        xn[9 + i] = fma_(Real(prm.dt_over_m), fs[i], x[9 + i]);
    }
    xn[11] += Real(prm.dt_g);
#pragma unroll
    for (int i = 0; i < NX; ++i) x[i] = xn[i];
}

}
```

### optistate_b200/csrc/kf_seq_tma.cuh

```cuda
#pragma once

#include <cuda.h>

#include "kf_seq_core.cuh"

namespace okf {

#ifndef OKF_BLK_WARPS
#define OKF_BLK_WARPS 4
#endif
template <bool kBlock>
__host__ __device__ constexpr int tma_warps() { return kBlock ? OKF_BLK_WARPS : 4; }
template <bool kBlock>
__host__ __device__ constexpr int tma_threads() { return 32 * tma_warps<kBlock>(); }
constexpr int TMA_CH_G0 = 24, TMA_CH_G1 = 10;
constexpr int TMA_CH_REF = 3;
constexpr int TMA_NOISE_ROWS = 22;
constexpr int TMA_NOISE_ROWS_OUT = 32;
template <int kW>
__host__ __device__ constexpr int tma_stages() { return kW == 1 ? 2 : 1; }
template <int kOut>
__host__ __device__ constexpr int tma_noise_rows() { return kOut != 0 ? TMA_NOISE_ROWS_OUT : TMA_NOISE_ROWS; }
constexpr int TMA_ACC_ROWS = 25;

__device__ __forceinline__ uint32_t smem_u32(const void *p) { return (uint32_t)__cvta_generic_to_shared(p); }
__device__ __forceinline__ void mbar_init(uint64_t *bar, uint32_t count) {
    asm volatile("mbarrier.init.shared::cta.b64 [%0], %1;" ::"r"(smem_u32(bar)), "r"(count) : "memory");
}
__device__ __forceinline__ void mbar_expect_tx(uint64_t *bar, uint32_t bytes) {
    asm volatile("mbarrier.arrive.expect_tx.shared::cta.b64 _, [%0], %1;" ::"r"(smem_u32(bar)), "r"(bytes) : "memory");
}
__device__ __forceinline__ void mbar_wait(uint64_t *bar, uint32_t parity) {
    uint32_t done;
    do {
        asm volatile(
            "{\n .reg .pred p;\n mbarrier.try_wait.parity.shared::cta.b64 p, [%1], %2;\n selp.u32 %0, 1, 0, p;\n}"
            : "=r"(done)
            : "r"(smem_u32(bar)), "r"(parity)
            : "memory");
    } while (!done);
}
__device__ __forceinline__ void bulk_g2s(void *dst, const void *src, uint32_t bytes, uint64_t *bar) {
    asm volatile("cp.async.bulk.shared::cluster.global.mbarrier::complete_tx::bytes [%0], [%1], %2, [%3];" ::"r"(smem_u32(dst)),
                 "l"(src), "r"(bytes), "r"(smem_u32(bar))
                 : "memory");
}

struct alignas(64) TmaMaps {
    CUtensorMap p, f, z, lab0, lab1, body_ref;
};

__device__ __forceinline__ void tma_tile_g2s(void *dst, const CUtensorMap *map, int col, int row, uint64_t *bar) {
    asm volatile("cp.async.bulk.tensor.2d.shared::cluster.global.tile.mbarrier::complete_tx::bytes [%0], [%1, {%2, %3}], [%4];" ::"r"(
                     smem_u32(dst)),
                 "l"(map), "r"(col), "r"(row), "r"(smem_u32(bar))
                 : "memory");
}

template <typename Real, int kThreads, int kNoiseRows = TMA_NOISE_ROWS, int kStages = 1>
struct TmaSmem {
    static __host__ __device__ constexpr size_t warp_rows(int n_lab, int ref_rows) { return TMA_CH_G0 + TMA_CH_G1 + 12 * n_lab + ref_rows; }
    static __host__ __device__ constexpr size_t warp_bytes(int n_lab, int ref_rows) { return warp_rows(n_lab, ref_rows) * 32 * sizeof(Real); }
    static __host__ __device__ constexpr size_t off_in() { return 128; }
    static __host__ __device__ constexpr size_t off_noise(int n_lab, int ref_rows) { return off_in() + kStages * warp_bytes(n_lab, ref_rows); }
    static __host__ __device__ constexpr size_t off_acc(int n_lab, int ref_rows) { return off_noise(n_lab, ref_rows) + (size_t)kNoiseRows * kThreads * sizeof(Real); }
    static __host__ __device__ constexpr size_t total(int n_lab, int ref_rows, bool acc_in_smem) {
        return off_acc(n_lab, ref_rows) + (acc_in_smem ? (size_t)TMA_ACC_ROWS * kThreads * 8 : 0);
    }
};

template <bool kMpc, typename Real>
__device__ __forceinline__ void issue_g0(const TmaMaps &m, long long t, int s_warp, Real *g0w, Real *refw, uint64_t *bar, int lane) {
    if (lane == 0) {
        mbar_expect_tx(bar, (uint32_t)((TMA_CH_G0 + (kMpc ? TMA_CH_REF : 0)) * 32 * sizeof(Real)));
        tma_tile_g2s(g0w, &m.p, s_warp, (int)(t * 12), bar);
        tma_tile_g2s(g0w + 12 * 32, &m.f, s_warp, (int)(t * 12), bar);
        if constexpr (kMpc) tma_tile_g2s(refw, &m.body_ref, s_warp, (int)(t * 12), bar);
    }
}
template <typename Real>
__device__ __forceinline__ void issue_g1(const TmaMaps &m, long long t, int s_warp, Real *g1w, uint64_t *bar, int lane) {
    if (lane == 0) {
        mbar_expect_tx(bar, (uint32_t)(TMA_CH_G1 * 32 * sizeof(Real)));
        tma_tile_g2s(g1w, &m.z, s_warp, (int)(t * 10), bar);
    }
}
template <typename Real>
__device__ __forceinline__ void issue_g2(const TmaMaps &m, long long t, int s_warp, int n_lab, Real *g2w, uint64_t *bar, int lane) {
    if (lane == 0) {
        mbar_expect_tx(bar, (uint32_t)(12 * n_lab * 32 * sizeof(Real)));
        tma_tile_g2s(g2w, &m.lab0, s_warp, (int)(t * 12), bar);
        if (n_lab > 1) tma_tile_g2s(g2w + 12 * 32, &m.lab1, s_warp, (int)(t * 12), bar);
    }
}

template <typename Real, bool kSummary, bool kBlock>
__host__ __device__ constexpr int tma_min_blocks() {
#ifdef OKF_BLK_MINB
    if (kBlock) return OKF_BLK_MINB;
#endif
    if (kBlock) return (sizeof(Real) == 8 || kSummary) ? 3 : 4;
    return (sizeof(Real) == 4 && !kSummary) ? 3 : 2;
}
template <typename Real, bool kSummary, bool kBlock>
__host__ __device__ constexpr bool tma_acc_in_smem() {
#ifdef OKF_BLK_ACC_SMEM
    if (kBlock) return kSummary && sizeof(Real) == 8 && OKF_BLK_ACC_SMEM;
#endif
    return kSummary && sizeof(Real) == 8;
}

template <typename Real, bool kSummary, int kOut, bool kMpc, bool kBlock = false, int kW = 0>
__global__ void __launch_bounds__(kW ? 32 * kW : tma_threads<kBlock>(), kW == 1 ? 1 : tma_min_blocks<Real, kSummary, kBlock>()) kf_seq_tma_kernel(const __grid_constant__ Params<typename Lanes<Real>::scalar> prm,
                                                                 const __grid_constant__ TmaMaps maps) {
    using Scalar = typename Lanes<Real>::scalar;
    using AccT = typename Acc<Real>::type;
    constexpr int L = Lanes<Real>::n;
    static_assert(!(kBlock && kMpc), "the element-wise exponential of predict_mpc couples every state");
    constexpr bool kAccSmem = kW == 1 ? false : tma_acc_in_smem<Real, kSummary, kBlock>();
    extern __shared__ __align__(128) unsigned char smem_raw[];
    constexpr int TMA_WARPS = kW ? kW : tma_warps<kBlock>(), nt = 32 * TMA_WARPS;
    constexpr int kStages = tma_stages<kW>();
    using Smem = TmaSmem<Real, nt, tma_noise_rows<kOut>(), kStages>;
    const int tid = threadIdx.x, lane = tid & 31, warp = tid >> 5;
    const long long N = prm.N, S = prm.S;
    constexpr int TW = 32 * L;
    const long long n_pass = (N + S - 1) / S;
    const long long groups = (n_pass + TMA_WARPS - 1) / TMA_WARPS;
    const long long tile_k = blockIdx.x / groups, grp_j = blockIdx.x % groups;
    const long long m_pass = grp_j * TMA_WARPS + warp;
    const bool warp_active = m_pass < n_pass;
    const int n_active = (int)(n_pass - grp_j * TMA_WARPS < TMA_WARPS ? n_pass - grp_j * TMA_WARPS : TMA_WARPS);
    const long long i = m_pass * S + tile_k * TW + (long long)lane * L;
    const bool active = warp_active && i < N;
    const long long ic = active ? i : N - L;
    const int s_warp = (int)((tile_k * TW + prm.stream_offset) % S);
    const int n_lab = kSummary ? (prm.truth ? 1 : 0) + (prm.nominal ? 1 : 0) : 0;

    uint64_t *bars = reinterpret_cast<uint64_t *>(smem_raw);
    int *consumed = reinterpret_cast<int *>(smem_raw + 64);
    constexpr int kRefRows = kMpc ? TMA_CH_REF : 0;
    Real *g0w = reinterpret_cast<Real *>(smem_raw + Smem::off_in());
    Real *g1w = g0w + TMA_CH_G0 * 32, *g2w = g1w + TMA_CH_G1 * 32;
    Real *refw = g2w + 12 * n_lab * 32;
    Real *noise = reinterpret_cast<Real *>(smem_raw + Smem::off_noise(n_lab, kRefRows));
    AccT *acc_s = reinterpret_cast<AccT *>(smem_raw + Smem::off_acc(n_lab, kRefRows)) + tid;

    if (grp_j * TMA_WARPS * S + tile_k * TW >= N) return;
    const int tile_elems = (int)Smem::warp_rows(n_lab, kRefRows) * 32;
    if (tid == 0) {
#pragma unroll
        for (int b = 0; b < 3 * kStages; ++b) mbar_init(&bars[b], 1);
        consumed[0] = consumed[1] = consumed[2] = 0;
        asm volatile("fence.mbarrier_init.release.cluster;" ::: "memory");
    }
    __syncthreads();
    if (!warp_active) return;
    if (prm.T > 0 && warp == 0) {
#pragma unroll
        for (int sg = 0; sg < kStages; ++sg) {
            if (sg < prm.T) {
                issue_g0<kMpc>(maps, sg, s_warp, g0w + sg * tile_elems, refw + sg * tile_elems, &bars[3 * sg], lane);
                issue_g1(maps, sg, s_warp, g1w + sg * tile_elems, &bars[3 * sg + 1], lane);
                if (n_lab) issue_g2(maps, sg, s_warp, n_lab, g2w + sg * tile_elems, &bars[3 * sg + 2], lane);
            }
        }
    }
    const auto last_reader = [&](int g) -> int {
        __syncwarp();
        int last = 0;
        if constexpr (TMA_WARPS == 1) {
            if (lane == 0) __threadfence_block();
            return lane == 0 ? 0 : 1;
        }
        if (lane == 0) {
            __threadfence_block();
            last = atomicAdd(&consumed[g], 1) == n_active - 1;
            if (last) {
                consumed[g] = 0;
                __threadfence_block();
            }
        }
        return last ? 0 : 1;
    };

    Real *q = noise + tid, *r = noise + 12 * nt + tid;
#pragma unroll
    for (int c = 0; c < NX; ++c) q[c * nt] = prm.q_kind == OPTI_KF_MAT_DIAG ? Real(prm.Q[c]) : ld_traj(prm.Q, c * N + ic, Real());
#pragma unroll
    for (int c = 0; c < NZ; ++c) r[c * nt] = prm.r_kind == OPTI_KF_MAT_DIAG ? Real(prm.R[c]) : ld_traj(prm.R, c * N + ic, Real());
    if constexpr (kOut != 0) {
#pragma unroll
        for (int c = 0; c < NZ; ++c) r[(NZ + c) * nt] = rcp_(r[c * nt]);
    }
    Real x[NX], P[NP];
#pragma unroll
    for (int c = 0; c < NX; ++c) x[c] = prm.x0_inc ? ld_traj(prm.x0, c * prm.x0_ld + ic, Real()) : Real(prm.x0[c]);
#pragma unroll
    for (int a = 0; a < NX; ++a)
#pragma unroll
        for (int b = 0; b <= a; ++b) {
            Real v = Real(0);
            if (cpl<kBlock>(a, b)) switch (prm.p0_kind) {
                case OPTI_KF_MAT_NONE: v = (a == b) ? q[a * nt] : Real(0); break;
                case OPTI_KF_MAT_DIAG: v = (a == b) ? Real(prm.P0[a]) : Real(0); break;
                case OPTI_KF_MAT_DIAG_PER: v = (a == b) ? ld_traj(prm.P0, a * N + ic, Real()) : Real(0); break;
                case OPTI_KF_MAT_DENSE: v = Real(prm.P0[a * NX + b]); break;
                default: v = ld_traj(prm.P0, (long long)(a * NX + b) * N + ic, Real()); break;
            }
            P[tri(a, b)] = v;
        }

    uint32_t status[L];
#pragma unroll
    for (int ln = 0; ln < L; ++ln) status[ln] = 0;
    Real ptrace = Real(0), kgain = Real(0), ymax = Real(0);
    constexpr int kAccRegs = (kSummary && !kAccSmem) ? TMA_ACC_ROWS : 1;
    AccT acc_r[kAccRegs];
#pragma unroll
    for (int c = 0; c < kAccRegs; ++c) acc_r[c] = acc_zero(AccT());
    auto acc_add = [&](int idx, AccT v) {
        if constexpr (kAccSmem) acc_s[idx * nt] = acc_s[idx * nt] + v;
        else if constexpr (kSummary) acc_r[idx] = acc_r[idx] + v;
    };
    auto acc_get = [&](int idx) -> AccT {
        if constexpr (kAccSmem) return acc_s[idx * nt];
        else if constexpr (kSummary) return acc_r[idx];
        else return acc_zero(AccT());
    };
    if constexpr (kSummary) {
#pragma unroll
        for (int c = 0; c < TMA_ACC_ROWS; ++c) {
            if constexpr (kAccSmem) acc_s[c * nt] = acc_zero(AccT()); else acc_r[c] = acc_zero(AccT());
        }
    }

    const Real *lab_truth = (kSummary && prm.truth) ? g2w + lane : g0w + lane;
    const Real *lab_nominal = (kSummary && prm.nominal) ? g2w + (prm.truth ? 12 * 32 : 0) + lane : g0w + lane;
    auto accumulate = [&](int acc0, const Real *lab) {
#pragma unroll
        for (int c0 = 0; c0 < NX; c0 += 6) {
            Real lv[6];
#pragma unroll
            for (int c = 0; c < 6; ++c) lv[c] = lab[(c0 + c) * 32];
            if constexpr (kAccSmem) {
                AccT av[6];
#pragma unroll
                for (int c = 0; c < 6; ++c) av[c] = acc_s[(acc0 + c0 + c) * nt];
#pragma unroll
                for (int c = 0; c < 6; ++c) acc_s[(acc0 + c0 + c) * nt] = err_acc(av[c], x[c0 + c], lv[c]);
            } else if constexpr (kSummary) {
#pragma unroll
                for (int c = 0; c < 6; ++c) acc_r[acc0 + c0 + c] = err_acc(acc_r[acc0 + c0 + c], x[c0 + c], lv[c]);
            }
        }
    };
    auto trace_of = [](const Real (&Pm)[NP]) {
        Real h[6];
#pragma unroll
        for (int c = 0; c < 6; ++c) h[c] = Pm[tri(2 * c, 2 * c)] + Pm[tri(2 * c + 1, 2 * c + 1)];
        return ((h[0] + h[1]) + (h[2] + h[3])) + (h[4] + h[5]);
    };

    const Real e1_mpc = kMpc ? exp_minus_one(Real(prm.dt)) : Real(0);
    Real Rm[9];
    rot_zyx(x[0], x[1], x[2], Rm);
    bool any_trunc = may_truncate(Rm);

    for (long long t = 0; t < prm.T; ++t) {
        const int stg = kStages == 2 ? (int)(t & 1) * tile_elems : 0;
        const uint32_t par = kStages == 2 ? (uint32_t)((t >> 1) & 1) : (uint32_t)(t & 1);
        const bool more = t + kStages < prm.T;
        uint64_t *bar = bars + (kStages == 2 ? 3 * (int)(t & 1) : 0);
        Real *g0 = g0w + stg, *g1 = g1w + stg, *g2 = g2w + stg, *rf = refw + stg;

        mbar_wait(&bar[0], par);
        propagate_mean_with_R<32>(prm, x, g0 + lane, g0 + 12 * 32 + lane, Rm, any_trunc,
                              (kOut == 2 && active) ? prm.p_world_steps : nullptr, (t * 12) * N + i, N);
        Real E[kMpc ? 9 : 1];
        if constexpr (kMpc) {
            Real Rb[9];
            rot_zyx(rf[lane], rf[32 + lane], rf[64 + lane], Rb);
#pragma unroll
            for (int a = 0; a < 3; ++a)
#pragma unroll
                for (int k = 0; k < 3; ++k) E[3 * a + k] = exp_minus_one(Real(prm.dt) * Rb[3 * k + a]);
        }
        {
            const int elect = last_reader(0);
            if (more) issue_g0<kMpc>(maps, t + kStages, s_warp, g0, rf, &bar[0], elect);
        }
        if constexpr (kOut == 2) {
            if (active && prm.x_model_steps) {
#pragma unroll
                for (int c = 0; c < NX; ++c) st_traj(prm.x_model_steps, (t * NX + c) * N + i, x[c]);
            }
        }

        if constexpr (kMpc) cov_predict_mpc_sym(P, E, e1_mpc, q, nt);
        else cov_predict_sym<kBlock>(P, Rm, prm.dt, q, nt);

        mbar_wait(&bar[1], par);
        if constexpr (kSummary) {
            if (n_lab) mbar_wait(&bar[2], par);
        }
        const Real *z = g1 + lane;
        if constexpr (kOut == 2) {
            if (active && prm.z_steps) {
#pragma unroll
                for (int c = 0; c < NZ; ++c) st_traj(prm.z_steps, (t * NZ + c) * N + i, z[c * 32]);
            }
        }
        Real nis = Real(0), inv, inv_n;
        {
            const Real s = P[tri(0, 0)] + r[0];
            note_bad_pivot(s, status, OPTI_KF_ST_NOT_PD);
            inv = rcp_(s);
        }
        auto nothing = [] {};
        fold_pipelined<0, kBlock>(P, x, z[0 * 32], r[0 * nt], r[1 * nt], inv, inv_n, nis, status, nothing); inv = inv_n;
        fold_pipelined<1, kBlock>(P, x, z[1 * 32], r[1 * nt], r[2 * nt], inv, inv_n, nis, status, nothing); inv = inv_n;
        fold_pipelined<2, kBlock>(P, x, z[2 * 32], r[2 * nt], r[3 * nt], inv, inv_n, nis, status, nothing); inv = inv_n;
        fold_pipelined<3, kBlock>(P, x, z[3 * 32], r[3 * nt], r[4 * nt], inv, inv_n, nis, status, nothing); inv = inv_n;
        fold_pipelined<4, kBlock>(P, x, z[4 * 32], r[4 * nt], r[5 * nt], inv, inv_n, nis, status, nothing); inv = inv_n;
        fold_pipelined<5, kBlock>(P, x, z[5 * 32], r[5 * nt], r[6 * nt], inv, inv_n, nis, status, nothing); inv = inv_n;
        fold_pipelined<6, kBlock>(P, x, z[6 * 32], r[6 * nt], r[7 * nt], inv, inv_n, nis, status, nothing); inv = inv_n;
        fold_pipelined<7, kBlock>(P, x, z[7 * 32], r[7 * nt], r[8 * nt], inv, inv_n, nis, status, nothing); inv = inv_n;
        fold_pipelined<8, kBlock>(P, x, z[8 * 32], r[8 * nt], r[9 * nt], inv, inv_n, nis, status, nothing); inv = inv_n;
        const Real z9 = z[9 * 32], r9 = r[9 * nt];
        {
            const int elect = last_reader(1);
            if (more) issue_g1(maps, t + kStages, s_warp, g1, &bar[1], elect);
        }
        fold_pipelined<9, kBlock>(P, x, z9, r9, r9, inv, inv_n, nis, status, [&] {
            rot_zyx(x[0], x[1], x[2], Rm);
            any_trunc = may_truncate(Rm);
            if constexpr (kSummary) {
                accumulate(0, lab_truth + stg);
                accumulate(12, lab_nominal + stg);
            }
        });

        ymax = max_(ymax, nis);

        if constexpr (kOut != 0) {
            ptrace = trace_of(P);
            if (prm.k_gain_steps != nullptr) kgain = gain_trace_rinv<kBlock>(P, r + NZ * nt, nt);
            if (active) {
                if (prm.x_steps) {
#pragma unroll
                    for (int c = 0; c < NX; ++c) st_traj(prm.x_steps, (t * NX + c) * N + i, x[c]);
                }
                if (prm.p_trace_steps) st_traj(prm.p_trace_steps, t * N + i, ptrace);
                if (prm.k_gain_steps) st_traj(prm.k_gain_steps, t * N + i, kgain);
                if (prm.nis_steps) st_traj(prm.nis_steps, t * N + i, nis);
                if constexpr (kOut == 2) {
                    if (prm.P_ckpt && prm.ckpt_every > 0 && (t + 1) % prm.ckpt_every == 0) {
                        const long long base = ((t + 1) / prm.ckpt_every - 1) * (long long)(NX * NX) * N + i;
#pragma unroll
                        for (int a = 0; a < NX; ++a)
#pragma unroll
                            for (int b = 0; b < NX; ++b) st_traj(prm.P_ckpt, base + (long long)(a * NX + b) * N, cpl<kBlock>(a, b) ? P[tri(a, b)] : Real(0));
                    }
                }
            }
        }

        if constexpr (kSummary) {
            acc_add(24, to_acc(nis));
            if (n_lab) {
                const int elect = last_reader(2);
                if (more) issue_g2(maps, t + kStages, s_warp, n_lab, g2, &bar[2], elect);
            }
        }
    }

#pragma unroll
    for (int c = 0; c < NX; ++c) note_nonfinite(x[c], status, OPTI_KF_ST_NONFINITE);
    if (!active) return;
    if (prm.x_final) {
#pragma unroll
        for (int c = 0; c < NX; ++c) st_traj(prm.x_final, c * N + i, x[c]);
    }
    if (prm.P_final) {
#pragma unroll
        for (int a = 0; a < NX; ++a)
#pragma unroll
            for (int b = 0; b < NX; ++b) st_traj(prm.P_final, (long long)(a * NX + b) * N + i, cpl<kBlock>(a, b) ? P[tri(a, b)] : Real(0));
    }
    if (kSummary && prm.summary) {
        if (prm.T > 0) {
            ptrace = trace_of(P);
            kgain = gain_trace<kBlock>(P, r, nt);
        }
        const double invT = prm.T > 0 ? 1.0 / (double)prm.T : 0.0;
#pragma unroll
        for (int c = 0; c < NX; ++c) {
            st_summary(prm, c, i, x[c]);
            st_summary(prm, 12 + c, i, P[tri(c, c)]);
            st_summary(prm, 24 + c, i, prm.truth ? rms_out(acc_get(c), invT, Real()) : Real(0));
            st_summary(prm, 36 + c, i, prm.nominal ? rms_out(acc_get(12 + c), invT, Real()) : Real(0));
        }
        st_summary(prm, 48, i, mean_out(acc_get(24), invT, Real()));
        st_summary(prm, 49, i, ptrace);
        st_summary(prm, 50, i, kgain);
        st_summary(prm, 51, i, sqrt_(ymax));
    }
    if (prm.status) {
#pragma unroll
        for (int ln = 0; ln < L; ++ln)
            prm.status[i + ln] = status[ln] | (prm.stream_status ? prm.stream_status[s_warp + lane * L + ln] : 0u);
    }
}

}
```

### optistate_b200/csrc/kf_seq_tma_host.cuh

```cuda
#pragma once

#include <cuda.h>

#include <cstring>

#include "kf_launch.cuh"
#include "kf_seq_tma.cuh"

namespace okf {

using EncodeTiledFn = CUresult (*)(CUtensorMap *, CUtensorMapDataType, cuuint32_t, void *, const cuuint64_t *, const cuuint64_t *,
                                   const cuuint32_t *, const cuuint32_t *, CUtensorMapInterleave, CUtensorMapSwizzle,
                                   CUtensorMapL2promotion, CUtensorMapFloatOOBfill);
inline EncodeTiledFn encode_tiled() {
    static const EncodeTiledFn fn = [] {
        void *sym = nullptr;
        cudaDriverEntryPointQueryResult q;
        if (cudaGetDriverEntryPoint("cuTensorMapEncodeTiled", &sym, cudaEnableDefault, &q) != cudaSuccess || q != cudaDriverEntryPointSuccess)
            sym = nullptr;
        return (EncodeTiledFn)sym;
    }();
    return fn;
}

template <typename Real>
bool make_map(CUtensorMap *m, const Real *base, long long T, int C, long long S, int box_w, int rows) {
    EncodeTiledFn enc = encode_tiled();
    if (!enc || !base) return false;
    const cuuint64_t gdim[2] = {(cuuint64_t)S, (cuuint64_t)(T * C)};
    const cuuint64_t gstride[1] = {(cuuint64_t)S * sizeof(Real)};
    const cuuint32_t box[2] = {(cuuint32_t)box_w, (cuuint32_t)rows};
    const cuuint32_t estride[2] = {1u, 1u};
    return enc(m, sizeof(Real) == 8 ? CU_TENSOR_MAP_DATA_TYPE_FLOAT64 : CU_TENSOR_MAP_DATA_TYPE_FLOAT32, 2, (void *)base, gdim, gstride,
               box, estride, CU_TENSOR_MAP_INTERLEAVE_NONE, CU_TENSOR_MAP_SWIZZLE_NONE, CU_TENSOR_MAP_L2_PROMOTION_L2_128B,
               CU_TENSOR_MAP_FLOAT_OOB_FILL_NONE) == CUDA_SUCCESS;
}

template <typename Real, bool kSummary, int kOut, bool kMpc, bool kBlock, int kW = 0>
int launch_seq_tma_k(const Params<typename Lanes<Real>::scalar> &p, cudaStream_t stream) {
    constexpr int L = Lanes<Real>::n;
    const int n_lab = kSummary ? (p.truth ? 1 : 0) + (p.nominal ? 1 : 0) : 0;
    TmaMaps maps;
    std::memset(&maps, 0, sizeof maps);
    const int bw = 32 * L;
    bool ok = make_map(&maps.p, p.p, p.T, 12, p.S, bw, 12) && make_map(&maps.f, p.f, p.T, 12, p.S, bw, 12) &&
              make_map(&maps.z, p.z_in, p.T, 10, p.S, bw, 10);
    if (ok && kMpc) ok = make_map(&maps.body_ref, p.body_ref, p.T, 12, p.S, bw, 3);
    if (ok && n_lab >= 1) ok = make_map(&maps.lab0, p.truth ? p.truth : p.nominal, p.T, 12, p.S, bw, 12);
    if (ok && n_lab >= 2) ok = make_map(&maps.lab1, p.nominal, p.T, 12, p.S, bw, 12);
    if (!ok) return 1;
    constexpr int kWarps = kW ? kW : tma_warps<kBlock>(), kThreads = 32 * kWarps;
    const size_t smem = TmaSmem<Real, kThreads, tma_noise_rows<kOut>(), tma_stages<kW>()>::total(n_lab, kMpc ? TMA_CH_REF : 0, kW == 1 ? false : tma_acc_in_smem<Real, kSummary, kBlock>());
    auto kern = kf_seq_tma_kernel<Real, kSummary, kOut, kMpc, kBlock, kW>;
    if (cudaFuncSetAttribute(kern, cudaFuncAttributeMaxDynamicSharedMemorySize, (int)smem) != cudaSuccess) return OPTI_KF_E_CUDA;
    const long long tiles = p.S / (32 * L), n_pass = (p.N + p.S - 1) / p.S;
    const long long blocks = tiles * ((n_pass + kWarps - 1) / kWarps);
    if (blocks > 0x7fffffffLL) return OPTI_KF_E_SHAPE;
    kern<<<(unsigned)blocks, kThreads, smem, stream>>>(p, maps);
    return OPTI_KF_OK;
}

template <typename Real, bool kSummary, bool kBlock>
int launch_seq_tma(const Params<typename Lanes<Real>::scalar> &p, cudaStream_t stream) {
    const bool rare = p.x_model_steps || p.p_world_steps || p.z_steps || p.P_ckpt;
    const bool estimates = p.x_steps || p.p_trace_steps || p.k_gain_steps || p.nis_steps;
    const int out = rare ? 2 : (estimates ? 1 : 0);
    const bool mpc = p.cov_model == OPTI_KF_COV_MPC;
    if constexpr (kBlock) {
        if (mpc) return OPTI_KF_E_UNSUPPORTED;
        switch (out) {
            case 0: return launch_seq_tma_k<Real, kSummary, 0, false, true>(p, stream);
            case 1: return launch_seq_tma_k<Real, kSummary, 1, false, true>(p, stream);
            default: return launch_seq_tma_k<Real, kSummary, 2, false, true>(p, stream);
        }
    } else {
        switch (out * 2 + (mpc ? 1 : 0)) {
            case 0: return launch_seq_tma_k<Real, kSummary, 0, false, false>(p, stream);
            case 1: return launch_seq_tma_k<Real, kSummary, 0, true, false>(p, stream);
            case 2: return launch_seq_tma_k<Real, kSummary, 1, false, false>(p, stream);
            case 3: return launch_seq_tma_k<Real, kSummary, 1, true, false>(p, stream);
            case 4: return launch_seq_tma_k<Real, kSummary, 2, false, false>(p, stream);
            default: return launch_seq_tma_k<Real, kSummary, 2, true, false>(p, stream);
        }
    }
}

template <typename Real, bool kSummary>
int launch_seq_tma_lone(const Params<typename Lanes<Real>::scalar> &p, cudaStream_t stream) {
    const bool rare = p.x_model_steps || p.p_world_steps || p.z_steps || p.P_ckpt;
    const bool estimates = p.x_steps || p.p_trace_steps || p.k_gain_steps || p.nis_steps;
    if (rare) return launch_seq_tma_k<Real, kSummary, 2, false, true, 1>(p, stream);
    if (estimates) return launch_seq_tma_k<Real, kSummary, 1, false, true, 1>(p, stream);
    return launch_seq_tma_k<Real, kSummary, 0, false, true, 1>(p, stream);
}

}
```

### optistate_b200/pipeline.py

```python
from __future__ import annotations

from typing import Dict, Sequence

import torch

from . import _native as nv
from .batch import kf_batch

_STREAM_CH = {"imu": 6, "p": 12, "dp": 12, "contact": 4, "f": 12, "truth": 12, "nominal": 12}


def stream_share_plan(sizes: Dict[str, int], world: int, rank: int):
    ranges, off = {}, 0
    for k, n in sizes.items():
        ranges[k] = (off, off + int(n))
        off += int(n)
    flat_len = (off + world - 1) // world * world
    share = flat_len // world
    c0, c1 = rank * share, (rank + 1) * share
    pieces = []
    for k, (a, b) in ranges.items():
        lo, hi = max(a, c0), min(b, c1)
        if lo < hi:
            pieces.append((k, lo - a, lo, hi - lo))
    return flat_len, ranges, pieces


class KfHostPipeline:
    def __init__(self, n_traj: int, n_steps: int, n_streams: int, *, dtype: torch.dtype = torch.float64,
                 labels: Sequence[str] = ("truth", "nominal"), stream_offset: int = 0, n_slots: int = 2, device=None,
                 structure: str = "auto", shared_streams_group=None, trace: bool = False):
        nv.require_cuda()
        self.device = torch.device("cuda", torch.cuda.current_device()) if device is None else torch.device(device)
        self.n_traj, self.n_steps, self.n_streams, self.dtype = n_traj, n_steps, n_streams, dtype
        self.labels, self.stream_offset, self.n_slots = tuple(labels), int(stream_offset), n_slots
        self.structure = structure
        esz = 8 if dtype == torch.float64 else 4
        names = ["imu", "p", "dp", "contact", "f", *self.labels]
        self.group, self.world, self.rank = shared_streams_group, 1, 0
        if shared_streams_group is not None:
            import torch.distributed as dist

            self.world, self.rank = dist.get_world_size(shared_streams_group), dist.get_rank(shared_streams_group)
        self._flat_len, self._ranges, self._pieces = stream_share_plan({k: n_steps * _STREAM_CH[k] * n_streams for k in names}, self.world, self.rank)
        self.h2d_bytes_per_batch = 0
        self.slots = []
        for _ in range(n_slots):
            flat = torch.empty(self._flat_len, dtype=dtype, device=self.device)
            dev = {k: flat[a:b].view(n_steps, _STREAM_CH[k], n_streams) for k, (a, b) in self._ranges.items()}
            dev["Q"] = torch.empty((12, n_traj), dtype=dtype, device=self.device)
            dev["R"] = torch.empty((10, n_traj), dtype=dtype, device=self.device)
            out = {"summary": torch.empty((nv.SUMMARY_ROWS, n_traj), dtype=dtype, device=self.device),
                   "status": torch.zeros(n_traj, dtype=torch.int32, device=self.device),
                   "workspace": torch.empty(n_steps * 10 * n_streams * esz + 4 * n_streams + 4096, dtype=torch.uint8, device=self.device)}
            host = torch.empty((nv.SUMMARY_ROWS, n_traj), dtype=dtype).pin_memory()
            self.slots.append({"dev": dev, "flat": flat, "out": out, "host": host, "ev_in": torch.cuda.Event(), "ev_k": torch.cuda.Event(),
                               "ev_out": torch.cuda.Event(), "busy": False})
        self.s_in, self.s_k, self.s_out = (torch.cuda.Stream(device=self.device) for _ in range(3))
        self._next = 0
        self._trace = [] if trace else None

    def submit(self, host: Dict[str, torch.Tensor]) -> int:
        i = self._next
        self._next = (self._next + 1) % self.n_slots
        slot = self.slots[i]
        if slot["busy"]:
            slot["ev_out"].synchronize()
        dev = slot["dev"]
        tr = None
        if self._trace is not None:
            tr = {k: torch.cuda.Event(enable_timing=True) for k in ("in0", "in1", "in2", "k0", "k1", "o1")}
            self._trace.append(tr)
        with torch.cuda.stream(self.s_in):
            if slot["busy"]:
                self.s_in.wait_event(slot["ev_k"])
            if tr:
                tr["in0"].record(self.s_in)
            copied = 0
            if self.world == 1:
                for k, d in dev.items():
                    d.copy_(host[k], non_blocking=True)
                    copied += d.numel()
            else:
                import torch.distributed as dist

                flat, share = slot["flat"], self._flat_len // self.world
                c0, c1 = self.rank * share, (self.rank + 1) * share
                for k, src0, dst0, cnt in self._pieces:
                    flat[dst0:dst0 + cnt].copy_(host[k].reshape(-1)[src0:src0 + cnt], non_blocking=True)
                    copied += cnt
                for k in ("Q", "R"):
                    dev[k].copy_(host[k], non_blocking=True)
                    copied += dev[k].numel()
                if tr:
                    tr["in1"].record(self.s_in)
                dist.all_gather_into_tensor(flat, flat[c0:c1], group=self.group)
            self.h2d_bytes_per_batch = copied * (8 if self.dtype == torch.float64 else 4)
            slot["ev_in"].record(self.s_in)
            if tr:
                tr["in2"].record(self.s_in)
        with torch.cuda.stream(self.s_k):
            self.s_k.wait_event(slot["ev_in"])
            if tr:
                tr["k0"].record(self.s_k)
            kf_batch(dev["imu"], dev["p"], dev["dp"], dev["contact"], dev["f"], Q=dev["Q"], R=dev["R"], n_traj=self.n_traj,
                     dtype=self.dtype, stream_offset=self.stream_offset, truth=dev.get("truth"), nominal=dev.get("nominal"),
                     outputs=("summary",), out=slot["out"], q_kind=nv.MAT_DIAG_PER, r_kind=nv.MAT_DIAG_PER, device=self.device,
                     structure=self.structure)
            slot["ev_k"].record(self.s_k)
            if tr:
                tr["k1"].record(self.s_k)
        with torch.cuda.stream(self.s_out):
            self.s_out.wait_event(slot["ev_k"])
            slot["host"].copy_(slot["out"]["summary"], non_blocking=True)
            slot["ev_out"].record(self.s_out)
            if tr:
                tr["o1"].record(self.s_out)
        slot["busy"] = True
        return i

    def result(self, ticket: int) -> torch.Tensor:
        slot = self.slots[ticket]
        slot["ev_out"].synchronize()
        return slot["host"]

    def drain(self):
        for slot in self.slots:
            if slot["busy"]:
                slot["ev_out"].synchronize()

    def timeline(self):
        if not self._trace:
            return []
        self.drain()
        torch.cuda.synchronize(self.device)
        base = self._trace[0]["in0"]
        out = []
        for tr in self._trace:
            row = {}
            for k, ev in tr.items():
                try:
                    row[k] = round(base.elapsed_time(ev), 2)
                except Exception:
                    row[k] = None
            out.append(row)
        return out
```

Baseline: 19.02 billion.

## Precompute per-stream leg moments in measure kernel to shrink TMA per-step inputs

The per-stream quantities (outer products p_i f_j summed over legs, plus the force sums) are computed once per stream and time step in the measure pre-pass and stored in the workspace. The sequential TMA kernel then loads 12 moment rows instead of 24 rows of p and f, and rebuilds the torque from R and the moments. Many trajectories share each stream, so this removes repeated loads and arithmetic from the per-trajectory loop. The cost is a larger workspace, extra global writes in the pre-pass, and slightly different rounding in the torque because of the reassociation.

Result: faster. 20.46 billion, median of 6 (+7.6%).

```diff
diff --git a/optistate_b200/batch.py b/optistate_b200/batch.py
--- a/optistate_b200/batch.py
+++ b/optistate_b200/batch.py
@@ -205,6 +205,8 @@
             ws = out.get("workspace") if out is not None else None
             if ws is None or ws.numel() < ws_bytes:
                 ws = torch.empty(int(ws_bytes), dtype=torch.uint8, device=device)
+                if out is not None:
+                    out["workspace"] = ws
             tensors["workspace"] = ws
         nv.check(int(ext.kf_batch(cfg, consts, tensors)), "optistate_kf_batch")
     res = {k: tensors[k] for k in want}
diff --git a/optistate_b200/csrc/kf_abi.cu b/optistate_b200/csrc/kf_abi.cu
--- a/optistate_b200/csrc/kf_abi.cu
+++ b/optistate_b200/csrc/kf_abi.cu
@@ -6,6 +6,7 @@
 #include "kf_identify.cuh"
 #include "kf_launch.cuh"
 #include "kf_mpc_params.cuh"
+#include "kf_seq_core.cuh"
 
 namespace {
 
@@ -86,17 +87,22 @@
 }
 
 template <typename Real>
-void launch_measure(long long T, long long S, const Real *imu, const Real *p, const Real *dp, const Real *contact, Real *z,
-                    Real *odom, uint32_t *status, cudaStream_t stream);
+void launch_measure(long long T, long long S, const Real *imu, const Real *p, const Real *dp, const Real *contact, const Real *f, Real *z,
+                    Real *mom, Real *odom, uint32_t *status, cudaStream_t stream);
 
 inline bool aligned16(const void *p) { return (reinterpret_cast<uintptr_t>(p) & 15u) == 0; }
 
-size_t seq_workspace_bytes(const OptiKfDesc *d) {
-    if (d->phases != OPTI_KF_PHASE_ALL) return 0;
-    const size_t esz = d->dtype == OPTI_KF_F64 ? 8 : 4;
-    const size_t z_bytes = ((size_t)d->n_steps * okf::NZ * (size_t)d->n_streams * esz + 255) & ~(size_t)255;
-    return z_bytes + (((size_t)d->n_streams * sizeof(uint32_t) + 255) & ~(size_t)255);
-}
+struct SeqWorkspace {
+    size_t mom, status, total;
+    explicit SeqWorkspace(const OptiKfDesc *d) {
+        const auto up = [](size_t b) { return (b + 255) & ~(size_t)255; };
+        const size_t esz = d->dtype == OPTI_KF_F64 ? 8 : 4, ts = (size_t)d->n_steps * (size_t)d->n_streams;
+        const bool all = d->phases == OPTI_KF_PHASE_ALL;
+        mom = all ? up(ts * okf::NZ * esz) : 0;
+        status = mom + up(ts * okf::NM * esz);
+        total = status + (all ? up((size_t)d->n_streams * sizeof(uint32_t)) : 0);
+    }
+};
 
 bool tma_layout_ok(const OptiKfDesc *d) {
     if (d->stream_index != nullptr || d->n_steps == 0) return false;
@@ -154,23 +160,25 @@
         p.stream_status = d->status;
     }
     if (algo == OPTI_KF_ALGO_SEQUENTIAL) {
-        bool streamed = tma_layout_ok(d);
-        if (streamed && d->phases == OPTI_KF_PHASE_ALL) {
-            const size_t need = seq_workspace_bytes(d);
-            if (d->workspace && d->workspace_bytes >= need && aligned16(d->workspace)) {
-                const size_t esz = sizeof(Real);
-                const size_t z_bytes = ((size_t)d->n_steps * okf::NZ * (size_t)d->n_streams * esz + 255) & ~(size_t)255;
-                Real *z = (Real *)d->workspace;
-                uint32_t *sst = (uint32_t *)((unsigned char *)d->workspace + z_bytes);
-                if (cudaMemsetAsync(sst, 0, (size_t)d->n_streams * sizeof(uint32_t), stream) != cudaSuccess) return OPTI_KF_E_CUDA;
-                launch_measure<Real>(d->n_steps, d->n_streams, p.imu, p.p, p.dp, p.contact, z, nullptr, sst, stream);
-                p.z_in = z;
-                p.stream_status = sst;
+        bool streamed = tma_layout_ok(d) && (d->phases == OPTI_KF_PHASE_ALL || aligned16(p.z_in));
+        if (streamed) {
+            const SeqWorkspace ws(d);
+            if (d->workspace && d->workspace_bytes >= ws.total && aligned16(d->workspace)) {
+                unsigned char *base = (unsigned char *)d->workspace;
+                Real *z = nullptr;
+                uint32_t *sst = nullptr;
+                if (d->phases == OPTI_KF_PHASE_ALL) {
+                    z = (Real *)base;
+                    sst = (uint32_t *)(base + ws.status);
+                    if (cudaMemsetAsync(sst, 0, (size_t)d->n_streams * sizeof(uint32_t), stream) != cudaSuccess) return OPTI_KF_E_CUDA;
+                    p.z_in = z;
+                    p.stream_status = sst;
+                }
+                p.mom = (Real *)(base + ws.mom);
+                launch_measure<Real>(d->n_steps, d->n_streams, p.imu, p.p, p.dp, p.contact, p.f, z, (Real *)p.mom, nullptr, sst, stream);
             } else {
                 streamed = false;
             }
-        } else if (streamed && !aligned16(p.z_in)) {
-            streamed = false;
         }
         if (streamed) {
             const int rc = launch_streamed<Real>(d, p, stream);
@@ -193,38 +201,52 @@
 template <typename Real>
 __global__ void __launch_bounds__(256) kf_measure_kernel(long long T, long long S, const Real *__restrict__ imu,
                                                          const Real *__restrict__ p, const Real *__restrict__ dp,
-                                                         const Real *__restrict__ contact, Real *__restrict__ z,
+                                                         const Real *__restrict__ contact, const Real *__restrict__ f,
+                                                         Real *__restrict__ z, Real *__restrict__ mom,
                                                          Real *__restrict__ odom, uint32_t *__restrict__ status) {
     const long long idx = (long long)blockIdx.x * blockDim.x + threadIdx.x;
     if (idx >= T * S) return;
     const long long t = idx / S, s = idx % S;
-    Real im[6], pp[12], dd[12], cc[4], zz[okf::NZ];
-#pragma unroll
-    for (int c = 0; c < 6; ++c) im[c] = imu[(t * 6 + c) * S + s];
-#pragma unroll
-    for (int c = 0; c < 12; ++c) { pp[c] = p[(t * 12 + c) * S + s]; dd[c] = dp[(t * 12 + c) * S + s]; }
-#pragma unroll
-    for (int c = 0; c < 4; ++c) cc[c] = contact[(t * 4 + c) * S + s];
-    const bool all_swing = okf::form_measurement(im, pp, dd, cc, zz);
-    if (z) {
-#pragma unroll
-        for (int c = 0; c < okf::NZ; ++c) z[(t * okf::NZ + c) * S + s] = zz[c];
-    }
-    if (odom) {
-        odom[(t * 4 + 0) * S + s] = zz[3];
-        odom[(t * 4 + 1) * S + s] = zz[7];
-        odom[(t * 4 + 2) * S + s] = zz[8];
-        odom[(t * 4 + 3) * S + s] = zz[9];
-    }
-    if (status && all_swing) atomicOr(status + s, (uint32_t)OPTI_KF_ST_ALL_SWING);
-}
-
-template <typename Real>
-void launch_measure(long long T, long long S, const Real *imu, const Real *p, const Real *dp, const Real *contact, Real *z,
-                    Real *odom, uint32_t *status, cudaStream_t stream) {
+    Real pp[12];
+#pragma unroll
+    for (int c = 0; c < 12; ++c) pp[c] = p[(t * 12 + c) * S + s];
+    if (z || odom || status) {
+        Real im[6], dd[12], cc[4], zz[okf::NZ];
+#pragma unroll
+        for (int c = 0; c < 6; ++c) im[c] = imu[(t * 6 + c) * S + s];
+#pragma unroll
+        for (int c = 0; c < 12; ++c) dd[c] = dp[(t * 12 + c) * S + s];
+#pragma unroll
+        for (int c = 0; c < 4; ++c) cc[c] = contact[(t * 4 + c) * S + s];
+        const bool all_swing = okf::form_measurement(im, pp, dd, cc, zz);
+        if (z) {
+#pragma unroll
+            for (int c = 0; c < okf::NZ; ++c) z[(t * okf::NZ + c) * S + s] = zz[c];
+        }
+        if (odom) {
+            odom[(t * 4 + 0) * S + s] = zz[3];
+            odom[(t * 4 + 1) * S + s] = zz[7];
+            odom[(t * 4 + 2) * S + s] = zz[8];
+            odom[(t * 4 + 3) * S + s] = zz[9];
+        }
+        if (status && all_swing) atomicOr(status + s, (uint32_t)OPTI_KF_ST_ALL_SWING);
+    }
+    if (mom) {
+        Real ff[12], M[okf::NM];
+#pragma unroll
+        for (int c = 0; c < 12; ++c) ff[c] = f[(t * 12 + c) * S + s];
+        okf::leg_moments(pp, ff, M);
+#pragma unroll
+        for (int c = 0; c < okf::NM; ++c) mom[(t * okf::NM + c) * S + s] = M[c];
+    }
+}
+
+template <typename Real>
+void launch_measure(long long T, long long S, const Real *imu, const Real *p, const Real *dp, const Real *contact, const Real *f, Real *z,
+                    Real *mom, Real *odom, uint32_t *status, cudaStream_t stream) {
     const long long total = T * S;
     if (total == 0) return;
-    kf_measure_kernel<Real><<<(unsigned)((total + 255) / 256), 256, 0, stream>>>(T, S, imu, p, dp, contact, z, odom, status);
+    kf_measure_kernel<Real><<<(unsigned)((total + 255) / 256), 256, 0, stream>>>(T, S, imu, p, dp, contact, f, z, mom, odom, status);
     g_launches.fetch_add(1, std::memory_order_relaxed);
 }
 
@@ -308,7 +330,7 @@
     if (!bytes_out) return OPTI_KF_E_NULL;
     const int algo = resolve(desc);
     if (algo < 0) return algo;
-    *bytes_out = (algo == OPTI_KF_ALGO_SEQUENTIAL && tma_layout_ok(desc)) ? seq_workspace_bytes(desc) : 0;
+    *bytes_out = (algo == OPTI_KF_ALGO_SEQUENTIAL && tma_layout_ok(desc)) ? SeqWorkspace(desc).total : 0;
     return OPTI_KF_OK;
 }
 
@@ -343,10 +365,10 @@
     cudaGetLastError();
     if (d->dtype == OPTI_KF_F64)
         launch_measure<double>(d->n_steps, d->n_streams, (const double *)d->imu, (const double *)d->p, (const double *)d->dp,
-                               (const double *)d->contact, (double *)d->z, (double *)d->odom, d->status, stream);
+                               (const double *)d->contact, nullptr, (double *)d->z, nullptr, (double *)d->odom, d->status, stream);
     else
         launch_measure<float>(d->n_steps, d->n_streams, (const float *)d->imu, (const float *)d->p, (const float *)d->dp,
-                              (const float *)d->contact, (float *)d->z, (float *)d->odom, d->status, stream);
+                              (const float *)d->contact, nullptr, (float *)d->z, nullptr, (float *)d->odom, d->status, stream);
     return cudaGetLastError() == cudaSuccess ? OPTI_KF_OK : OPTI_KF_E_CUDA;
 }
 
diff --git a/optistate_b200/csrc/kf_closed_loop.cu b/optistate_b200/csrc/kf_closed_loop.cu
--- a/optistate_b200/csrc/kf_closed_loop.cu
+++ b/optistate_b200/csrc/kf_closed_loop.cu
@@ -10,7 +10,7 @@
 inline size_t up(size_t b) { return (b + kAlign - 1) & ~(kAlign - 1); }
 
 struct Layout {
-    size_t z, p0, p1, fh, wset, wmult, mst, total;
+    size_t z, p0, p1, fh, wset, wmult, mst, fws, total;
     Layout(int64_t N, int64_t T) {
         size_t o = 0;
         z = o; o += up((size_t)T * 10 * N * 8);
@@ -20,6 +20,7 @@
         wset = o; o += up((size_t)OPTI_KF_MPC_HORIZON * N * 4);
         wmult = o; o += up((size_t)OPTI_KF_MPC_HORIZON * 4 * 5 * N * 8);
         mst = o; o += up((size_t)N * 4);
+        fws = o; o += up((size_t)12 * N * 8);
         total = o;
     }
 };
@@ -89,6 +90,7 @@
     f.q_kind = d->q_kind; f.r_kind = d->r_kind; f.Q = d->Q; f.R = d->R;
     f.status = d->status;
     f.flags = d->status ? OPTI_KF_FLAG_STATUS_ACCUMULATE : 0;
+    f.workspace = ws + L.fws; f.workspace_bytes = L.total - L.fws;
 
     const double *x_cur = (const double *)d->x0;
     int x_per = d->x0_per_traj;
diff --git a/optistate_b200/csrc/kf_common.cuh b/optistate_b200/csrc/kf_common.cuh
--- a/optistate_b200/csrc/kf_common.cuh
+++ b/optistate_b200/csrc/kf_common.cuh
@@ -19,6 +19,7 @@
     int block;
     Real dt, dt_over_m, dt_g, inv_inertia[3];
     const Real *imu, *p, *dp, *contact, *f, *z_in, *body_ref, *truth, *nominal;
+    const Real *mom;
     const int32_t *stream_index;
     const Real *x0; long long x0_ld; int x0_inc;
     const Real *P0; int p0_kind;
diff --git a/optistate_b200/csrc/kf_seq.cuh b/optistate_b200/csrc/kf_seq.cuh
--- a/optistate_b200/csrc/kf_seq.cuh
+++ b/optistate_b200/csrc/kf_seq.cuh
@@ -73,7 +73,12 @@
             if (form_measurement(imu, pf, dp, contact, z)) status[0] |= OPTI_KF_ST_ALL_SWING;
         }
 
-        propagate_mean_with_R<1>(prm, x, pf, ff, Rm, any_trunc, prm.p_world_steps, (t * 12) * N + i, N);
+        if (prm.p_world_steps) store_world_feet<1>(pf, Rm, prm.p_world_steps, (t * 12) * N + i, N);
+        {
+            Real M[NM];
+            leg_moments(pf, ff, M);
+            propagate_mean_from_moments<1>(prm, x, M, Rm, any_trunc);
+        }
         if (prm.x_model_steps) {
 #pragma unroll
             for (int c = 0; c < NX; ++c) st_stream(prm.x_model_steps + (t * NX + c) * N + i, x[c]);
diff --git a/optistate_b200/csrc/kf_seq_core.cuh b/optistate_b200/csrc/kf_seq_core.cuh
--- a/optistate_b200/csrc/kf_seq_core.cuh
+++ b/optistate_b200/csrc/kf_seq_core.cuh
@@ -210,27 +210,40 @@
     return m >= (sizeof(S) == 8 ? 0x3ff00000 : 0x3f7ffff0);
 }
 
+constexpr int NM = 12;
+template <typename Real>
+__device__ __forceinline__ void leg_moments(const Real (&p)[12], const Real (&f)[12], Real (&M)[NM]) {
+#pragma unroll
+    for (int m = 0; m < 3; ++m)
+#pragma unroll
+        for (int k = 0; k < 3; ++k)
+            M[3 * m + k] = fma_(p[9 + m], f[9 + k], fma_(p[6 + m], f[6 + k], fma_(p[3 + m], f[3 + k], mul_rn(p[m], f[k]))));
+#pragma unroll
+    for (int k = 0; k < 3; ++k) M[9 + k] = ((f[k] + f[3 + k]) + f[6 + k]) + f[9 + k];
+}
+
 template <int STRIDE, typename Real, typename Scalar>
-__device__ __forceinline__ void propagate_mean_with_R(const Params<Scalar> &prm, Real (&x)[NX], const Real *pin, const Real *fin,
-                                                      const Real (&R)[9], bool any_trunc, Scalar *pw_out, long long pw_idx, long long pw_stride) {
-    constexpr int L = Lanes<Real>::n;
-    Real tau[3] = {Real(0), Real(0), Real(0)}, fs[3] = {Real(0), Real(0), Real(0)};
+__device__ __forceinline__ void store_world_feet(const Real *pin, const Real (&R)[9], Scalar *pw_out, long long pw_idx, long long pw_stride) {
 #pragma unroll
     for (int l = 0; l < 4; ++l) {
         const Real a = pin[(3 * l) * STRIDE], b = pin[(3 * l + 1) * STRIDE], c = pin[(3 * l + 2) * STRIDE];
-        const Real pw0 = fma_(R[2], c, fma_(R[1], b, R[0] * a));
-        const Real pw1 = fma_(R[5], c, fma_(R[4], b, R[3] * a));
-        const Real pw2 = fma_(R[8], c, fma_(R[7], b, R[6] * a));
-        if (pw_out) {
-            st_traj(pw_out, pw_idx + (3 * l) * pw_stride, pw0);
-            st_traj(pw_out, pw_idx + (3 * l + 1) * pw_stride, pw1);
-            st_traj(pw_out, pw_idx + (3 * l + 2) * pw_stride, pw2);
-        }
-        const Real f0 = fin[(3 * l) * STRIDE], f1 = fin[(3 * l + 1) * STRIDE], f2 = fin[(3 * l + 2) * STRIDE];
-        tau[0] += fnma_(pw2, f1, pw1 * f2);
-        tau[1] += fnma_(pw0, f2, pw2 * f0);
-        tau[2] += fnma_(pw1, f0, pw0 * f1);
-        fs[0] += f0; fs[1] += f1; fs[2] += f2;
+        st_traj(pw_out, pw_idx + (3 * l) * pw_stride, fma_(R[2], c, fma_(R[1], b, R[0] * a)));
+        st_traj(pw_out, pw_idx + (3 * l + 1) * pw_stride, fma_(R[5], c, fma_(R[4], b, R[3] * a)));
+        st_traj(pw_out, pw_idx + (3 * l + 2) * pw_stride, fma_(R[8], c, fma_(R[7], b, R[6] * a)));
+    }
+}
+
+template <int STRIDE, typename Real, typename Scalar>
+__device__ __forceinline__ void propagate_mean_from_moments(const Params<Scalar> &prm, Real (&x)[NX], const Real *min, const Real (&R)[9],
+                                                            bool any_trunc) {
+    constexpr int L = Lanes<Real>::n;
+    const auto C = [&](int k) { return min[k * STRIDE]; };
+    Real tau[3];
+#pragma unroll
+    for (int i = 0; i < 3; ++i) {
+        const int j = (i + 1) % 3, k = (i + 2) % 3;
+        tau[i] = fnma_(R[3 * k + 2], C(6 + j), fnma_(R[3 * k + 1], C(3 + j), fnma_(R[3 * k], C(j),
+                 fma_(R[3 * j + 2], C(6 + k), fma_(R[3 * j + 1], C(3 + k), mul_rn(R[3 * j], C(k)))))));
     }
     Real u[3];
 #pragma unroll
@@ -258,7 +271,7 @@
         xn[i] = x[i] + dth[i];
         xn[3 + i] = fma_(dt, x[9 + i], x[3 + i]);
         xn[6 + i] = fma_(dt, fma_(R[3 * i + 2], u[2], fma_(R[3 * i + 1], u[1], R[3 * i] * u[0])), x[6 + i]);
-        xn[9 + i] = fma_(Real(prm.dt_over_m), fs[i], x[9 + i]);
+        xn[9 + i] = fma_(Real(prm.dt_over_m), min[(9 + i) * STRIDE], x[9 + i]);
     }
     xn[11] += Real(prm.dt_g);
 #pragma unroll
diff --git a/optistate_b200/csrc/kf_seq_tma.cuh b/optistate_b200/csrc/kf_seq_tma.cuh
--- a/optistate_b200/csrc/kf_seq_tma.cuh
+++ b/optistate_b200/csrc/kf_seq_tma.cuh
@@ -13,8 +13,10 @@
 __host__ __device__ constexpr int tma_warps() { return kBlock ? OKF_BLK_WARPS : 4; }
 template <bool kBlock>
 __host__ __device__ constexpr int tma_threads() { return 32 * tma_warps<kBlock>(); }
-constexpr int TMA_CH_G0 = 24, TMA_CH_G1 = 10;
+constexpr int TMA_CH_G1 = 10;
 constexpr int TMA_CH_REF = 3;
+template <int kOut, bool kMpc>
+__host__ __device__ constexpr int tma_g0_rows() { return NM + (kOut == 2 ? 12 : 0) + (kMpc ? TMA_CH_REF : 0); }
 constexpr int TMA_NOISE_ROWS = 22;
 constexpr int TMA_NOISE_ROWS_OUT = 32;
 template <int kW>
@@ -47,7 +49,7 @@
 }
 
 struct alignas(64) TmaMaps {
-    CUtensorMap p, f, z, lab0, lab1, body_ref;
+    CUtensorMap mom, p, z, lab0, lab1, body_ref;
 };
 
 __device__ __forceinline__ void tma_tile_g2s(void *dst, const CUtensorMap *map, int col, int row, uint64_t *bar) {
@@ -59,23 +61,23 @@
 
 template <typename Real, int kThreads, int kNoiseRows = TMA_NOISE_ROWS, int kStages = 1>
 struct TmaSmem {
-    static __host__ __device__ constexpr size_t warp_rows(int n_lab, int ref_rows) { return TMA_CH_G0 + TMA_CH_G1 + 12 * n_lab + ref_rows; }
-    static __host__ __device__ constexpr size_t warp_bytes(int n_lab, int ref_rows) { return warp_rows(n_lab, ref_rows) * 32 * sizeof(Real); }
+    static __host__ __device__ constexpr size_t warp_rows(int n_lab, int g0_rows) { return g0_rows + TMA_CH_G1 + 12 * n_lab; }
+    static __host__ __device__ constexpr size_t warp_bytes(int n_lab, int g0_rows) { return warp_rows(n_lab, g0_rows) * 32 * sizeof(Real); }
     static __host__ __device__ constexpr size_t off_in() { return 128; }
-    static __host__ __device__ constexpr size_t off_noise(int n_lab, int ref_rows) { return off_in() + kStages * warp_bytes(n_lab, ref_rows); }
-    static __host__ __device__ constexpr size_t off_acc(int n_lab, int ref_rows) { return off_noise(n_lab, ref_rows) + (size_t)kNoiseRows * kThreads * sizeof(Real); }
-    static __host__ __device__ constexpr size_t total(int n_lab, int ref_rows, bool acc_in_smem) {
-        return off_acc(n_lab, ref_rows) + (acc_in_smem ? (size_t)TMA_ACC_ROWS * kThreads * 8 : 0);
+    static __host__ __device__ constexpr size_t off_noise(int n_lab, int g0_rows) { return off_in() + kStages * warp_bytes(n_lab, g0_rows); }
+    static __host__ __device__ constexpr size_t off_acc(int n_lab, int g0_rows) { return off_noise(n_lab, g0_rows) + (size_t)kNoiseRows * kThreads * sizeof(Real); }
+    static __host__ __device__ constexpr size_t total(int n_lab, int g0_rows, bool acc_in_smem) {
+        return off_acc(n_lab, g0_rows) + (acc_in_smem ? (size_t)TMA_ACC_ROWS * kThreads * 8 : 0);
     }
 };
 
-template <bool kMpc, typename Real>
-__device__ __forceinline__ void issue_g0(const TmaMaps &m, long long t, int s_warp, Real *g0w, Real *refw, uint64_t *bar, int lane) {
+template <int kOut, bool kMpc, typename Real>
+__device__ __forceinline__ void issue_g0(const TmaMaps &m, long long t, int s_warp, Real *g0w, uint64_t *bar, int lane) {
     if (lane == 0) {
-        mbar_expect_tx(bar, (uint32_t)((TMA_CH_G0 + (kMpc ? TMA_CH_REF : 0)) * 32 * sizeof(Real)));
-        tma_tile_g2s(g0w, &m.p, s_warp, (int)(t * 12), bar);
-        tma_tile_g2s(g0w + 12 * 32, &m.f, s_warp, (int)(t * 12), bar);
-        if constexpr (kMpc) tma_tile_g2s(refw, &m.body_ref, s_warp, (int)(t * 12), bar);
+        mbar_expect_tx(bar, (uint32_t)(tma_g0_rows<kOut, kMpc>() * 32 * sizeof(Real)));
+        tma_tile_g2s(g0w, &m.mom, s_warp, (int)(t * NM), bar);
+        if constexpr (kOut == 2) tma_tile_g2s(g0w + NM * 32, &m.p, s_warp, (int)(t * 12), bar);
+        if constexpr (kMpc) tma_tile_g2s(g0w + (tma_g0_rows<kOut, kMpc>() - TMA_CH_REF) * 32, &m.body_ref, s_warp, (int)(t * 12), bar);
     }
 }
 template <typename Real>
@@ -139,15 +141,14 @@
 
     uint64_t *bars = reinterpret_cast<uint64_t *>(smem_raw);
     int *consumed = reinterpret_cast<int *>(smem_raw + 64);
-    constexpr int kRefRows = kMpc ? TMA_CH_REF : 0;
+    constexpr int kG0Rows = tma_g0_rows<kOut, kMpc>();
     Real *g0w = reinterpret_cast<Real *>(smem_raw + Smem::off_in());
-    Real *g1w = g0w + TMA_CH_G0 * 32, *g2w = g1w + TMA_CH_G1 * 32;
-    Real *refw = g2w + 12 * n_lab * 32;
-    Real *noise = reinterpret_cast<Real *>(smem_raw + Smem::off_noise(n_lab, kRefRows));
-    AccT *acc_s = reinterpret_cast<AccT *>(smem_raw + Smem::off_acc(n_lab, kRefRows)) + tid;
+    Real *g1w = g0w + kG0Rows * 32, *g2w = g1w + TMA_CH_G1 * 32;
+    Real *noise = reinterpret_cast<Real *>(smem_raw + Smem::off_noise(n_lab, kG0Rows));
+    AccT *acc_s = reinterpret_cast<AccT *>(smem_raw + Smem::off_acc(n_lab, kG0Rows)) + tid;
 
     if (grp_j * TMA_WARPS * S + tile_k * TW >= N) return;
-    const int tile_elems = (int)Smem::warp_rows(n_lab, kRefRows) * 32;
+    const int tile_elems = (int)Smem::warp_rows(n_lab, kG0Rows) * 32;
     if (tid == 0) {
 #pragma unroll
         for (int b = 0; b < 3 * kStages; ++b) mbar_init(&bars[b], 1);
@@ -160,7 +161,7 @@
 #pragma unroll
         for (int sg = 0; sg < kStages; ++sg) {
             if (sg < prm.T) {
-                issue_g0<kMpc>(maps, sg, s_warp, g0w + sg * tile_elems, refw + sg * tile_elems, &bars[3 * sg], lane);
+                issue_g0<kOut, kMpc>(maps, sg, s_warp, g0w + sg * tile_elems, &bars[3 * sg], lane);
                 issue_g1(maps, sg, s_warp, g1w + sg * tile_elems, &bars[3 * sg + 1], lane);
                 if (n_lab) issue_g2(maps, sg, s_warp, n_lab, g2w + sg * tile_elems, &bars[3 * sg + 2], lane);
             }
@@ -272,15 +273,18 @@
         const uint32_t par = kStages == 2 ? (uint32_t)((t >> 1) & 1) : (uint32_t)(t & 1);
         const bool more = t + kStages < prm.T;
         uint64_t *bar = bars + (kStages == 2 ? 3 * (int)(t & 1) : 0);
-        Real *g0 = g0w + stg, *g1 = g1w + stg, *g2 = g2w + stg, *rf = refw + stg;
+        Real *g0 = g0w + stg, *g1 = g1w + stg, *g2 = g2w + stg;
 
         mbar_wait(&bar[0], par);
-        propagate_mean_with_R<32>(prm, x, g0 + lane, g0 + 12 * 32 + lane, Rm, any_trunc,
-                              (kOut == 2 && active) ? prm.p_world_steps : nullptr, (t * 12) * N + i, N);
+        if constexpr (kOut == 2) {
+            if (active && prm.p_world_steps) store_world_feet<32>(g0 + NM * 32 + lane, Rm, prm.p_world_steps, (t * 12) * N + i, N);
+        }
+        propagate_mean_from_moments<32>(prm, x, g0 + lane, Rm, any_trunc);
         Real E[kMpc ? 9 : 1];
         if constexpr (kMpc) {
             Real Rb[9];
-            rot_zyx(rf[lane], rf[32 + lane], rf[64 + lane], Rb);
+            const Real *rf = g0 + (kG0Rows - TMA_CH_REF) * 32 + lane;
+            rot_zyx(rf[0], rf[32], rf[64], Rb);
 #pragma unroll
             for (int a = 0; a < 3; ++a)
 #pragma unroll
@@ -288,7 +292,7 @@
         }
         {
             const int elect = last_reader(0);
-            if (more) issue_g0<kMpc>(maps, t + kStages, s_warp, g0, rf, &bar[0], elect);
+            if (more) issue_g0<kOut, kMpc>(maps, t + kStages, s_warp, g0, &bar[0], elect);
         }
         if constexpr (kOut == 2) {
             if (active && prm.x_model_steps) {
diff --git a/optistate_b200/csrc/kf_seq_tma_host.cuh b/optistate_b200/csrc/kf_seq_tma_host.cuh
--- a/optistate_b200/csrc/kf_seq_tma_host.cuh
+++ b/optistate_b200/csrc/kf_seq_tma_host.cuh
@@ -43,14 +43,14 @@
     TmaMaps maps;
     std::memset(&maps, 0, sizeof maps);
     const int bw = 32 * L;
-    bool ok = make_map(&maps.p, p.p, p.T, 12, p.S, bw, 12) && make_map(&maps.f, p.f, p.T, 12, p.S, bw, 12) &&
-              make_map(&maps.z, p.z_in, p.T, 10, p.S, bw, 10);
+    bool ok = make_map(&maps.mom, p.mom, p.T, NM, p.S, bw, NM) && make_map(&maps.z, p.z_in, p.T, 10, p.S, bw, 10);
+    if (ok && kOut == 2) ok = make_map(&maps.p, p.p, p.T, 12, p.S, bw, 12);
     if (ok && kMpc) ok = make_map(&maps.body_ref, p.body_ref, p.T, 12, p.S, bw, 3);
     if (ok && n_lab >= 1) ok = make_map(&maps.lab0, p.truth ? p.truth : p.nominal, p.T, 12, p.S, bw, 12);
     if (ok && n_lab >= 2) ok = make_map(&maps.lab1, p.nominal, p.T, 12, p.S, bw, 12);
     if (!ok) return 1;
     constexpr int kWarps = kW ? kW : tma_warps<kBlock>(), kThreads = 32 * kWarps;
-    const size_t smem = TmaSmem<Real, kThreads, tma_noise_rows<kOut>(), tma_stages<kW>()>::total(n_lab, kMpc ? TMA_CH_REF : 0, kW == 1 ? false : tma_acc_in_smem<Real, kSummary, kBlock>());
+    const size_t smem = TmaSmem<Real, kThreads, tma_noise_rows<kOut>(), tma_stages<kW>()>::total(n_lab, tma_g0_rows<kOut, kMpc>(), kW == 1 ? false : tma_acc_in_smem<Real, kSummary, kBlock>());
     auto kern = kf_seq_tma_kernel<Real, kSummary, kOut, kMpc, kBlock, kW>;
     if (cudaFuncSetAttribute(kern, cudaFuncAttributeMaxDynamicSharedMemorySize, (int)smem) != cudaSuccess) return OPTI_KF_E_CUDA;
     const long long tiles = p.S / (32 * L), n_pass = (p.N + p.S - 1) / p.S;
diff --git a/optistate_b200/pipeline.py b/optistate_b200/pipeline.py
--- a/optistate_b200/pipeline.py
+++ b/optistate_b200/pipeline.py
@@ -35,7 +35,6 @@
         self.n_traj, self.n_steps, self.n_streams, self.dtype = n_traj, n_steps, n_streams, dtype
         self.labels, self.stream_offset, self.n_slots = tuple(labels), int(stream_offset), n_slots
         self.structure = structure
-        esz = 8 if dtype == torch.float64 else 4
         names = ["imu", "p", "dp", "contact", "f", *self.labels]
         self.group, self.world, self.rank = shared_streams_group, 1, 0
         if shared_streams_group is not None:
@@ -51,8 +50,7 @@
             dev["Q"] = torch.empty((12, n_traj), dtype=dtype, device=self.device)
             dev["R"] = torch.empty((10, n_traj), dtype=dtype, device=self.device)
             out = {"summary": torch.empty((nv.SUMMARY_ROWS, n_traj), dtype=dtype, device=self.device),
-                   "status": torch.zeros(n_traj, dtype=torch.int32, device=self.device),
-                   "workspace": torch.empty(n_steps * 10 * n_streams * esz + 4 * n_streams + 4096, dtype=torch.uint8, device=self.device)}
+                   "status": torch.zeros(n_traj, dtype=torch.int32, device=self.device)}
             host = torch.empty((nv.SUMMARY_ROWS, n_traj), dtype=dtype).pin_memory()
             self.slots.append({"dev": dev, "flat": flat, "out": out, "host": host, "ev_in": torch.cuda.Event(), "ev_k": torch.cuda.Event(),
                                "ev_out": torch.cuda.Event(), "busy": False})
```
